# baek0203/multimodal_survival_prediction

Hardware: AMD Instinct MI355X
Metric: patients/sec per epoch (training epoch of the K-fold job: fwd + Cox + gate entropy + bwd + clip + Adam; HBM-resident cohort, batches gathered on the device inside the timed region -- the same epoch fed from pinned host memory over PCIe: config.h2d) (higher is better)
Workload: dtype f32

## Files before the change

### include/mmsurv.h

```cpp
#ifndef MMSURV_H
#define MMSURV_H
#include <stdint.h>
#include <stddef.h>

#ifndef HIP_INCLUDE_HIP_HIP_RUNTIME_API_H
typedef struct ihipStream_t* hipStream_t;
typedef struct ihipEvent_t* hipEvent_t;
#endif

#define MMS_OK 0
#define MMS_ERR_ARG (-1)
#define MMS_ERR_LAUNCH (-2)
#define MMS_MAX_GROUP 10

#ifdef __cplusplus
extern "C" {
#endif

typedef struct Dims3 { int D; int H; int W; } Dims3;

typedef struct MmsDnOpts {
    int out_features;
    int persist_b4;
    int persist_b3;
    int split_wgs;
    int conv1_ksplit;
    int conv1_small;
    int c1s_max_wgs;
    int conv1_small_bwd;
    int fuse_apply_rows;
    int conv3_small;
    int c3s_ring;
    int conv3_mt;
    int conv3_mt32_min;
    int conv3w_mt;
    int big_ng;
    int batch_w;
    int ms3_rows;
    int ms1_div;
    int c0_nwg;
    int c0f_nwg;
    int w2_packed;
    int trans_prepass;
    int fuse_layers;
    int wgrad_tab;
    int skip_dead_bwd;
    int c0_zero_skip;
    int dup_zero;
} MmsDnOpts;

typedef struct BnSrc {
    const double* sum;
    const double* sumsq;
    const float* rmean;
    const float* rvar;
    const float* gamma;
    const float* beta;
    float inv_count;
    float eps;
    int train;
    int nrep;
    int rep_stride;
} BnSrc;


typedef struct Conv1FwdP {
    const float* x; int ldx;
    int M;
    int K;
    const float* w;
    int N;
    float* y; int ldy;
    BnSrc bn;
    double* osum; double* osumsq;
    int pool;
    Dims3 in;
    int srep; int sstride;
    float* partial; int ksplit; unsigned* counters;
} Conv1FwdP;

typedef struct Conv3FwdP {
    const float* y1;
    const int* coords;
    Dims3 g; int M;
    const float* wp;
    float* out; int ldo;
    BnSrc bn;
    double* osum; double* osumsq;
    float* partial;
    int nsplit;
    int srep; int sstride;
    int wfrag;
    const unsigned* zwords; int zbps;
} Conv3FwdP;

typedef struct Conv0FwdP {
    const float* x;
    Dims3 in; Dims3 out;
    const int* coords;
    int M;
    const float* w;
    float* y;
    double* osum; double* osumsq;
    int srep; int sstride;
} Conv0FwdP;

typedef struct PoolFwdP {
    const float* y0; Dims3 in;
    Dims3 out; int B;
    float* slab; int ld;
    uint8_t* argmax;
    BnSrc bn;
    double* osum; double* osumsq;
    int srep; int sstride;
} PoolFwdP;

typedef struct PoolActP {
    const float* x; int ldx;
    int K;
    BnSrc bn;
    Dims3 in; int Mout;
    float* y; int ldy;
} PoolActP;

typedef struct HeadFwdP {
    const float* slab; int ld; int C; int B; int V;
    BnSrc bn;
    const float* w; const float* bias; int N;
    float* pooled;
    float* out; int ldo;
} HeadFwdP;

typedef struct BnBwd {
    const double* s1;
    const double* s2;
    int nrep; int rep_stride;
} BnBwd;

typedef struct Conv3BwdDataP {
    const float* dz; int lddz;
    const int* coords; Dims3 g; int M;
    const float* wpb;
    const float* y1;
    BnSrc bn;
    float* dbn;
    double* s1; double* s2;
    float* partial;
    int nsplit;
    int srep; int sstride;
    int wfrag;
    const unsigned* live;
} Conv3BwdDataP;

typedef struct Conv3BwdWP {
    const float* y1; const int* coords; Dims3 g; int M;
    BnSrc bn;
    const float* dz; int lddz;
    float* dw;
    int msplit;
    int dw_layout;
    const unsigned* live;
} Conv3BwdWP;

#define MMS_WGRAD_MAX_MODELS 5
#define MMS_WGRAD_MAX_MEMBERS 90
typedef struct MmsWgradModel {
    const void* tab;
    const float* slab;
    const float* dslab;
    const int* coords;
    const double* st_slab;
    int M; Dims3 g; int srep;
} MmsWgradModel;
typedef struct MmsWgradMember {
    float* dw2;
    float* dw1;
    float* dgamma2; float* dbeta2;
    int model; int layer;
} MmsWgradMember;
typedef struct MmsWgradShape {
    int ld; int C0;
    int ms3; int ms1;
    int dw_layout;
    int count;
} MmsWgradShape;

typedef struct Conv1BwdP {
    const float* dyraw; int lddy;
    const float* y; int ldy;
    BnSrc bn_out; BnBwd bb_out; int has_bn_out;
    int M; int N;
    const float* x; int ldx; int K; BnSrc bn_in;
    const float* w;
    int pool; Dims3 in;
    float* dw;
    float* dbn; int lddbn;
    double* s1; double* s2;
    int msplit;
    float* dgamma_out; float* dbeta_out;
    int srep; int sstride;
    float* fuse_dx; int fuse_lddx; int fuse_accumulate;
    float* fuse_dgamma; float* fuse_dbeta;
    const unsigned* live;
} Conv1BwdP;

typedef struct BnBwdApplyP {
    const float* dbn; int lddbn;
    const float* x; int ldx;
    float* dx; int lddx;
    int M; int C; BnSrc bn; BnBwd bb; int accumulate;
    float* dgamma; float* dbeta;
    const unsigned* live;
} BnBwdApplyP;

typedef struct HeadBwdP {
    const float* dout; int lddout;
    const float* pooled;
    const float* slab; int ld; int C; int B; int V; BnSrc bn;
    const float* w; int N;
    float* dw; float* dbias;
    float* dgamma; float* dbeta;
    float* dslab; int ldd;
    double* ext_sums;
} HeadBwdP;

typedef struct PoolBwdP {
    const float* dslab; int ld;
    const uint8_t* argmax; Dims3 out; Dims3 in; int B;
    const float* y0; BnSrc bn;
    float* dbn;
    double* s1; double* s2;
    const int* coords;
    int srep; int sstride;
} PoolBwdP;

typedef struct Conv0BwdWP {
    const float* dbn; const float* y0; BnSrc bn; BnBwd bb;
    const float* x; Dims3 in; Dims3 out; const int* coords; int M;
    float* dw; int msplit;
    float* dgamma; float* dbeta;
    float* dw_rep; int nrep;
    const unsigned* live;
} Conv0BwdWP;

typedef struct Conv0BwdDataP {
    const float* dbn;
    BnSrc bn;
    const float* w;
    Dims3 in; Dims3 out;
    int M;
    float* dx;
} Conv0BwdDataP;

typedef struct FbConvP {
    const float* x; int Cin; Dims3 in; Dims3 out; int B;
    int has_bn; BnSrc bn;
    const float* w; const float* bias; int Cout;
    float* y;
    double* osum; double* osumsq;
    const float* dy;
    float* dw; float* dbias;
    float* dbn_in; double* s1; double* s2;
    int msplit;
} FbConvP;

typedef struct FbPoolP {
    const float* y; int C; int V; int B; BnSrc bn;
    float* out; int ldo;
    const float* dout; int lddout;
    float* dbn; double* s1; double* s2;
} FbPoolP;

typedef struct InProlog {
    int bn;
    const float* gamma; const float* beta;
    float* rmean; float* rvar; long long* nbt;
    float eps; float momentum;
    int train;
    float drop_p;
    const float* drop_mask;
    const uint32_t* rng;
    uint32_t stream_id;
} InProlog;

typedef struct LinearFwdP {
    const float* x; int ldx; int M; int K;
    InProlog pro;
    const float* w; const float* bias; int N;
    float* y; int ldy; int out_relu;
} LinearFwdP;

typedef struct LinearBwdP {
    const float* dy; int lddy;
    const float* y; int ldy;
    int out_relu;
    const float* x; int ldx; int M; int K; InProlog pro;
    const float* w; int N;
    float* dw; float* dbias;
    float* dx; int lddx;
    float* dgamma; float* dbeta;
} LinearBwdP;

typedef struct GateP {
    const float* feats; const float* mask; int M;
    const float* w1; const float* b1; const float* w2; const float* b2;
    float* hidden;
    float* gate;
    float* fused;
    const float* dfused;
    float ent_weight;
    const float* dgate_ext;
    float* dfeats;
    float* dw1; float* db1; float* dw2; float* db2;
    float* entropy;
// ... 90 lines not shown
typedef struct AugRec {
    int flip;
    int dz; int dy; int dx;
    float scale; float offset;
    int drop;
    int reserved;
} AugRec;
#define MMS_AUG_PLAIN 0
#define MMS_AUG_VOLUME 1
#define MMS_AUG_MASK 2
typedef struct AugP {
    const AugRec* rec;
    int role[8];
    int drop_bit[8];
    int D; int H; int W;
    int max_shift[3];
} AugP;

typedef struct AffRec {
    float m[12];
    float sigma;
    unsigned seed;
    int reserved[2];
} AffRec;
typedef struct AffP {
    const AffRec* rec;
    int stage_floats;
} AffP;

int mms_abi_sizeof(const char* name);
int mms_abi_version(void);

int mms_init_coords(int* coords, int B, int D, int H, int W, hipStream_t s);
int mms_conv0_fwd(const Conv0FwdP* p, hipStream_t s);
int mms_pool_fwd(const PoolFwdP* p, hipStream_t s);
int mms_conv1_fwd(const Conv1FwdP* p, hipStream_t s);
int mms_conv3_fwd(const Conv3FwdP* p, hipStream_t s);
int mms_head_fwd(const HeadFwdP* p, hipStream_t s);
int mms_conv3_bwd_data(const Conv3BwdDataP* p, hipStream_t s);
int mms_conv3_bwd_weight(const Conv3BwdWP* p, hipStream_t s);
int mms_conv1_bwd_data(const Conv1BwdP* p, hipStream_t s);
int mms_conv1_bwd_weight(const Conv1BwdP* p, hipStream_t s);
int mms_bn_bwd_apply(const BnBwdApplyP* p, hipStream_t s);
int mms_head_bwd(const HeadBwdP* p, hipStream_t s);
int mms_pool_bwd(const PoolBwdP* p, hipStream_t s);
int mms_conv0_bwd_weight(const Conv0BwdWP* p, hipStream_t s);
int mms_unpack_conv3_grads(const void* table_host, int nlayers, hipStream_t s);
int mms_pack_conv3(const float* w, float* wpf, float* wpb, hipStream_t s);
int mms_pack_conv3_frag(const float* w, float* wff, float* wfb, hipStream_t s);
int mms_pack_conv3_table(const void* table_dev, int nlayers, hipStream_t s);
int mms_bn_running_update(const void* table_dev, int n, float momentum, hipStream_t s);


int mms_fb_conv_fwd(const FbConvP* p, hipStream_t s);
int mms_fb_conv_bwd_w(const FbConvP* p, hipStream_t s);
int mms_fb_conv_bwd_x(const FbConvP* p, hipStream_t s);
int mms_fb_pool_fwd(const FbPoolP* p, hipStream_t s);
int mms_fb_pool_bwd(const FbPoolP* p, hipStream_t s);
int mms_fb_workspace_bytes(int B, int D, int H, int W, size_t* bytes);
int mms_fb_init(void* ws, int B, int D, int H, int W, const void* const* buffers, hipStream_t s);
int mms_fb_forward(void* ws, int B, int D, int H, int W, const float* x, const void* const* params,
                   const void* const* buffers, float* out, int ldo, int train, hipStream_t s);
int mms_fb_backward(void* ws, int B, int D, int H, int W, const float* x, const void* const* params,
                    const float* dout, int lddout, void* const* grads, hipStream_t s);
int mms_fb3_workspace_bytes(const int* widths, int B, int D, int H, int W, size_t* bytes);
int mms_fb3_init(void* ws, size_t ws_bytes, const int* widths, int B, int D, int H, int W, const void* const* buffers, hipStream_t s);
int mms_fb3_forward(void* ws, size_t ws_bytes, const int* widths, int B, int D, int H, int W, const float* x, const void* const* params,
                    const void* const* buffers, float* out, int ldo, int train, hipStream_t s);
int mms_fb3_backward(void* ws, size_t ws_bytes, const int* widths, int B, int D, int H, int W, const float* x, const void* const* params,
                     const float* dout, int lddout, void* const* grads, hipStream_t s);

int mms_conv0_bwd_data(const Conv0BwdDataP* p, hipStream_t s);
int mms_conv0_bwd_data_group(const Conv0BwdDataP* p, int ng, hipStream_t s);
int mms_dn121_input_grad(void* ws, int B, int D, int H, int W, const float* x, const void* const* params, const void* const* buffers,
                         const float* dout, int lddout, float* dx, const MmsDnOpts* opts, hipStream_t s);
int mms_fb3_input_grad(void* ws, size_t ws_bytes, const int* widths, int B, int D, int H, int W, const float* x, const void* const* params,
                       const void* const* buffers, const float* dout, int lddout, float* dx, hipStream_t s);
int mms_dn121_input_grad_group(int ng, void* const* ws, int B, int D, int H, int W, const float* const* x, const void* const* const* params,
                               const void* const* const* buffers, const float* const* dout, int lddout, float* const* dx,
                               const MmsDnOpts* opts, hipStream_t s);
int mms_fb3_input_grad_group(int ng, void* const* ws, size_t ws_bytes, const int* widths, int B, int D, int H, int W, const float* const* x,
                             const void* const* const* params, const void* const* const* buffers, const float* const* dout, int lddout,
                             float* const* dx, hipStream_t s);

typedef struct EnsP {
    const float* x[10];
    int K; size_t n;
    float* mean; float* spread;
} EnsP;
int mms_ensemble_reduce(const EnsP* p, hipStream_t s);

int mms_linear_fwd(const LinearFwdP* p, hipStream_t s);
int mms_linear_bwd(const LinearBwdP* p, hipStream_t s);
int mms_gate_fwd(const GateP* p, hipStream_t s);
int mms_gate_bwd(const GateP* p, hipStream_t s);
int mms_gate_entropy(const float* gate, int M, float scale, float* loss, float* dgate, hipStream_t s);
int mms_linear_big_fwd(const LinBigP* p, hipStream_t s);
int mms_linear_big_bwd_w(const LinBigP* p, hipStream_t s);
int mms_linear_big_bwd_x(const LinBigP* p, hipStream_t s);
int mms_bn1d_bwd_apply(const LinBigP* p, hipStream_t s);
int mms_missing_mix_fwd(const MixP* p, hipStream_t s);
int mms_missing_mix_bwd(const MixP* p, hipStream_t s);
int mms_cox_fwd_bwd(const CoxP* p, hipStream_t s);
int mms_moe_fwd(const MoeP* p, hipStream_t s);
int mms_moe_bwd(const MoeP* p, hipStream_t s);
int mms_cindex_counts(const CindexP* p, hipStream_t s);
int mms_grad_sumsq(const AdamP* p, hipStream_t s);
int mms_clip_adam(const AdamP* p, hipStream_t s);
int mms_w2_pack(const AdamP* p, hipStream_t s);

int mms_ablation_build(void);
int mms_dn121_workspace_bytes(int B, int D, int H, int W, size_t* bytes);
int mms_dn121_region(int B, int D, int H, int W, const char* name, int index, size_t* off, size_t* bytes);
int mms_dn121_init(void* ws, int B, int D, int H, int W, const void* const* params, const void* const* buffers, const MmsDnOpts* opts, hipStream_t s);
int mms_dn121_w2_fragmask(int B, int D, int H, int W, const MmsDnOpts* opts, uint64_t* mask);
int mms_dn121_forward(void* ws, int B, int D, int H, int W, const float* x, const void* const* params,
                      const void* const* buffers, float* out, int ldo, int train, const MmsDnOpts* opts, hipStream_t s);
int mms_dn121_backward(void* ws, int B, int D, int H, int W, const float* x, const void* const* params,
                       const float* dout, int lddout, void* const* grads, const MmsDnOpts* opts, hipStream_t s);
typedef int (*mms_sync_fn)(void* user, double* base, int nrep, long rep_stride, int ncols, long pair_stride, hipStream_t s);
int mms_dn121_init_sync(void* ws, int B, int D, int H, int W, const void* const* params, const void* const* buffers, int bn_world,
                        const MmsDnOpts* opts, hipStream_t s);
int mms_dn121_forward_sync(void* ws, int B, int D, int H, int W, const float* x, const void* const* params,
                           const void* const* buffers, float* out, int ldo, int bn_world, mms_sync_fn hook, void* user,
                           const MmsDnOpts* opts, hipStream_t s);
int mms_dn121_backward_stage(void* ws, int B, int D, int H, int W, const float* x, const void* const* params,
                             const float* dout, int lddout, void* const* grads, int block_hi, int block_lo,
                             int bn_world, mms_sync_fn hook, void* user, const MmsDnOpts* opts, hipStream_t s);
int mms_head_bwd_sums(const HeadBwdP* p, hipStream_t s);
int mms_head_bwd_apply(const HeadBwdP* p, hipStream_t s);
int mms_dn121_backward_mt(void* ws, int B, int D, int H, int W, const float* x, const void* const* params,
                          const float* dout, int lddout, void* const* grads, const MmsDnOpts* opts, hipStream_t s, hipStream_t side,
                          hipEvent_t ev_fork, hipEvent_t ev_join);

int mms_ct_preprocess(const float* x, int inD, int inH, int inW, float* out, int oD, int oH, int oW, float* scratch, hipStream_t s);
int mms_rna_log_zscore(const float* counts, float* out, int n, int g, hipStream_t s);

int mms_conv0_fwd_group(const Conv0FwdP* p, int ng, const MmsDnOpts* opts, hipStream_t s);
int mms_conv0_fwd_group_zw(const Conv0FwdP* p, unsigned* const* zwords, int ng, const MmsDnOpts* opts, hipStream_t s);
int mms_pool_fwd_group(const PoolFwdP* p, int ng, hipStream_t s);
int mms_pool_act_group(const PoolActP* p, int ng, hipStream_t s);
int mms_conv1_fwd_group(const Conv1FwdP* p, int ng, const MmsDnOpts* opts, hipStream_t s);
int mms_conv3_fwd_group(const Conv3FwdP* p, int ng, const MmsDnOpts* opts, hipStream_t s);
int mms_head_fwd_group(const HeadFwdP* p, int ng, hipStream_t s);
int mms_conv3_bwd_data_group(const Conv3BwdDataP* p, int ng, const MmsDnOpts* opts, hipStream_t s);
int mms_conv3_bwd_weight_group(const Conv3BwdWP* p, int ng, const MmsDnOpts* opts, hipStream_t s);
int mms_conv3_bwd_weight_msplit(int M, int members, const MmsDnOpts* opts);
int mms_conv1_bwd_data_group(const Conv1BwdP* p, int ng, const MmsDnOpts* opts, hipStream_t s);
int mms_conv1_bwd_weight_group(const Conv1BwdP* p, int ng, hipStream_t s);
int mms_wgrad_tab_group(const MmsWgradModel* models, int nmodels, const MmsWgradMember* members, int nmembers,
                        const MmsWgradShape* shape, int which, hipStream_t s);
int mms_bn_bwd_apply_group(const BnBwdApplyP* p, int ng, hipStream_t s);
int mms_head_bwd_group(const HeadBwdP* p, int ng, hipStream_t s);
int mms_pool_bwd_group(const PoolBwdP* p, int ng, hipStream_t s);
int mms_conv0_bwd_weight_group(const Conv0BwdWP* p, int ng, const MmsDnOpts* opts, hipStream_t s);
int mms_pack_conv3_table_group(const void* const* tables_dev, int ng, int nlayers, hipStream_t s);
int mms_pack_conv3_table_group_ex(const void* const* tables_dev, int ng, int nlayers, uint64_t fragmask, hipStream_t s);
int mms_bn_running_update_group(const void* const* tables_dev, int ng, int n, float momentum, hipStream_t s);
int mms_missing_mix_fwd_group(const MixP* p, int ng, hipStream_t s);
int mms_missing_mix_bwd_group(const MixP* p, int ng, hipStream_t s);
int mms_gather_rows_group(const GatherP* p, int ng, hipStream_t s);
int mms_gather_aug_group(const GatherP* p, const AugP* a, int ng, hipStream_t s);
int mms_gather_affine_group(const GatherP* p, const AugP* a, const AffP* f, int ng, hipStream_t s);
int mms_unpack_conv3_grads_group(const float* const* scratch, float* const* const* dw, int ng, int nlayers, hipStream_t s);
int mms_zero_regions_group(void* const* regions_dev, int ng, size_t bytes, hipStream_t s);
int mms_linear_fwd_group(const LinearFwdP* p, int ng, hipStream_t s);
int mms_linear_bwd_group(const LinearBwdP* p, int ng, hipStream_t s);
int mms_gate_fwd_group(const GateP* p, int ng, hipStream_t s);
int mms_gate_bwd_group(const GateP* p, int ng, hipStream_t s);
int mms_cox_fwd_bwd_group(const CoxP* p, int ng, hipStream_t s);
int mms_moe_fwd_group(const MoeP* p, int ng, hipStream_t s);
int mms_moe_bwd_group(const MoeP* p, int ng, hipStream_t s);
int mms_grad_sumsq_group(const AdamP* p, int ng, hipStream_t s);
int mms_clip_adam_group(const AdamP* p, int ng, hipStream_t s);
int mms_w2_pack_group(const AdamP* p, int ng, hipStream_t s);
int mms_dn121_forward_group(int ng, void* const* ws, int B, int D, int H, int W, const float* const* x,
                            const void* const* const* params, const void* const* const* buffers, float* const* out,
                            int ldo, int train, const MmsDnOpts* opts, hipStream_t s);
int mms_dn121_backward_group(int ng, void* const* ws, int B, int D, int H, int W, const float* const* x,
                             const void* const* const* params, const float* const* dout, int lddout,
                             void* const* const* grads, const MmsDnOpts* opts, hipStream_t s);

int mms_fb_conv_fwd_group(const FbConvP* p, int ng, hipStream_t s);
int mms_fb_conv_bwd_w_group(const FbConvP* p, int ng, hipStream_t s);
int mms_fb_conv_bwd_x_group(const FbConvP* p, int ng, hipStream_t s);
int mms_fb_pool_fwd_group(const FbPoolP* p, int ng, hipStream_t s);
int mms_fb_pool_bwd_group(const FbPoolP* p, int ng, hipStream_t s);
int mms_fb_forward_group(int ng, void* const* ws, int B, int D, int H, int W, const float* const* x,
                         const void* const* const* params, const void* const* const* buffers, float* const* out,
                         int ldo, int train, hipStream_t s);
int mms_fb_backward_group(int ng, void* const* ws, int B, int D, int H, int W, const float* const* x,
                          const void* const* const* params, const float* const* dout, int lddout,
                          void* const* const* grads, hipStream_t s);
int mms_fb3_forward_group(int ng, void* const* ws, size_t ws_bytes, const int* widths, int B, int D, int H, int W, const float* const* x,
                          const void* const* const* params, const void* const* const* buffers, float* const* out,
                          int ldo, int train, hipStream_t s);
int mms_fb3_backward_group(int ng, void* const* ws, size_t ws_bytes, const int* widths, int B, int D, int H, int W, const float* const* x,
                           const void* const* const* params, const float* const* dout, int lddout,
                           void* const* const* grads, hipStream_t s);
int mms_img_tail_fwd_group(const FbPoolP* pool, const LinearFwdP* l1, const LinearFwdP* l2, int ng, hipStream_t s);
int mms_img_tail_bwd_group(const FbPoolP* pool, const LinearBwdP* l1, const LinearBwdP* l2, int ng, hipStream_t s);
int mms_img_forward_group(int ng, void* const* ws, size_t ws_bytes, const int* widths, int B, int D, int H, int W, const float* const* x,
                          const void* const* const* params, const void* const* const* buffers, float* const* out,
                          int ldo, int train, const LinearFwdP* l1, const LinearFwdP* l2, hipStream_t s);
int mms_img_backward_group(int ng, void* const* ws, size_t ws_bytes, const int* widths, int B, int D, int H, int W, const float* const* x,
                           const void* const* const* params, void* const* const* grads, const LinearBwdP* l1, const LinearBwdP* l2,
                           hipStream_t s);

#ifdef __cplusplus
}
#endif
#endif
```

### multimodal_survival_prediction_amd/csrc/common.h

```cpp
#pragma once
#include <utility>
#include <hip/hip_runtime.h>
#include <atomic>
#include <mutex>
#include <stdint.h>
#include <stdio.h>

#include "../../include/mmsurv.h"

typedef float f32x16 __attribute__((ext_vector_type(16)));
typedef float f32x4 __attribute__((ext_vector_type(4)));

template <class P> struct Grp { P p[MMS_MAX_GROUP]; int zdim; };
template <class P> static inline bool grp_fill(Grp<P>& a, const P* pp, int ng, int zdim) {
    if (!pp || ng < 1 || ng > MMS_MAX_GROUP) return false;
    for (int g = 0; g < ng; ++g) a.p[g] = pp[g];
    a.zdim = zdim;
    return true;
}
#define MMS_SINGLE(name, T) extern "C" int name(const T* p, hipStream_t s) { return name##_group(p, 1, s); }
#define MMS_SINGLE_O(name, T) extern "C" int name(const T* p, hipStream_t s) { return name##_group(p, 1, nullptr, s); }
static inline MmsDnOpts mms_opts(const MmsDnOpts* o) { return o ? *o : MmsDnOpts{}; }


__device__ __forceinline__ void xcd_place(int& gi, int& bx) {
    gi = blockIdx.z; bx = blockIdx.x;
    if ((gridDim.x & 7) != 0) return;
    const int k = blockIdx.x & 7, per = gridDim.x >> 3, ng = gridDim.z;
    if (ng > 1 && ng <= 8 && (8 % ng) == 0) {
        const int X = 8 / ng, slots = per * ng, slot = (blockIdx.x >> 3) + per * blockIdx.z;
        gi = k / X; bx = (k % X) * slots + slot;
    } else {
        bx = k * per + (blockIdx.x >> 3);
    }
}

__device__ __forceinline__ void xcd_place_parts(int& gi, int& bx, int& X, int& q, int& sl) {
    gi = blockIdx.z; bx = blockIdx.x; X = 1; q = 0; sl = blockIdx.x;
    if ((gridDim.x & 7) != 0) return;
    const int k = blockIdx.x & 7, per = gridDim.x >> 3, ng = gridDim.z;
    if (ng > 1 && ng <= 8 && (8 % ng) == 0) {
        X = 8 / ng; q = k % X; sl = (blockIdx.x >> 3) + per * blockIdx.z;
        gi = k / X; bx = q * (per * ng) + sl;
    } else {
        X = 8; q = k; sl = blockIdx.x >> 3;
        bx = k * per + sl;
    }
}

struct DupPlan { unsigned dups; int rep; };
__device__ __forceinline__ unsigned dup_issue(const unsigned* zw, int B) {
    const int lane = threadIdx.x & 63;
    return (zw && lane < B) ? __hip_atomic_load(zw + lane, __ATOMIC_RELAXED, __HIP_MEMORY_SCOPE_AGENT) : 0xffffffffu;
}
__device__ __forceinline__ bool dup_resolve(unsigned word, unsigned zbps, int B, int tps, int mode, int X, int q, int sl, int& tile, DupPlan& pl) {
    pl.dups = 0; pl.rep = 0;
    const unsigned zmask = (unsigned)__builtin_amdgcn_readfirstlane((int)(unsigned)__ballot(word == zbps));
    if (__popc(zmask) < 2) return true;
    const int rep = __ffs((int)zmask) - 1;
    const unsigned dmask = zmask & ~(1u << rep);
    int s;
    if (mode == 1) {
        s = tile / tps;
        if ((dmask >> s) & 1u) return false;
    } else {
        const int ct = (B - __popc(dmask)) * tps;
        if (sl * X + q >= ct) return false;
        const int t = q * (ct / X) + (q < ct % X ? q : ct % X) + sl;
        int cs = t / tps;
        for (s = 0; s < B; ++s) {
            if ((dmask >> s) & 1u) continue;
            if (cs == 0) break;
            --cs;
        }
        tile = s * tps + t % tps;
    }
    if (s == rep) { pl.dups = dmask; pl.rep = rep; }
    return true;
}

__device__ __forceinline__ unsigned live_issue(const unsigned* w) {
    return w ? __hip_atomic_load(w, __ATOMIC_RELAXED, __HIP_MEMORY_SCOPE_AGENT) : 1u;
}
__device__ __forceinline__ bool live_dead(unsigned v) { return __builtin_amdgcn_readfirstlane(v) == 0u; }
struct LiveTab { const unsigned* w[MMS_MAX_GROUP]; };
static inline LiveTab live_tab(const unsigned* const* live, int ng) {
    LiveTab t{};
    for (int g = 0; live && g < ng && g < MMS_MAX_GROUP; ++g) t.w[g] = live[g];
    return t;
}
template <class P, class = void> struct has_live_word { static constexpr bool value = false; };
template <class P> struct has_live_word<P, decltype((void)std::declval<const P&>().live)> { static constexpr bool value = true; };
template <class P> __device__ __forceinline__ const unsigned* live_word_of(const P& p) {
    if constexpr (has_live_word<P>::value) return p.live; else return nullptr;
}

__device__ __forceinline__ bool syncthreads_any(bool flag, int (*vote)[4], int& par) {
    const int w = __ballot(flag) != 0ull;
    if ((threadIdx.x & 63) == 0) vote[par][threadIdx.x >> 6] = w;
    __syncthreads();
    const int4 v = *(const int4*)vote[par];
    par ^= 1;
    return __builtin_amdgcn_readfirstlane(v.x | v.y | v.z | v.w) != 0;
}

template <class F, int... T>
__device__ __forceinline__ void static_for_impl(F&& f, std::integer_sequence<int, T...>) { (f(std::integral_constant<int, T>{}), ...); }
template <int N, class F>
__device__ __forceinline__ void static_for(F&& f) { static_for_impl(f, std::make_integer_sequence<int, N>{}); }

__device__ __forceinline__ double* stat_rep(double* base, int nrep, int stride) {
    return (base && nrep > 1) ? base + (size_t)(blockIdx.x % nrep) * stride : base;
}
template <int NA, class V>
__device__ __forceinline__ void rep_add(const V* const (&a)[NA], int nrep, size_t stride_doubles, V (&s)[NA]) {
    for (int r0 = 1; r0 < nrep; r0 += 3) {
        V t[NA][3];
#pragma unroll
        for (int j = 0; j < 3; ++j) {
            const size_t o = (size_t)(r0 + j < nrep ? r0 + j : 0) * stride_doubles;
#pragma unroll
            for (int i = 0; i < NA; ++i) t[i][j] = *(const V*)((const double*)a[i] + o);
        }
#pragma unroll
        for (int j = 0; j < 3; ++j)
            if (r0 + j < nrep) {
#pragma unroll
                for (int i = 0; i < NA; ++i) s[i] += t[i][j];
            }
    }
}
__device__ __forceinline__ double rep_sum(const double* a, int c, int nrep, int stride) {
    double s[1] = {a[c]};
    const double* const p[1] = {a + c};
    rep_add(p, nrep, (size_t)stride, s);
    return s[0];
}

__device__ __forceinline__ void pstore(float* p, float v) { __hip_atomic_store(p, v, __ATOMIC_RELAXED, __HIP_MEMORY_SCOPE_AGENT); }
__device__ __forceinline__ float pload(const float* p) { return __hip_atomic_load(p, __ATOMIC_RELAXED, __HIP_MEMORY_SCOPE_AGENT); }
__device__ __forceinline__ bool tile_last_arriver(unsigned* counter, unsigned nsplit, int tid) {
    __shared__ unsigned s_last;
    asm volatile("s_waitcnt vmcnt(0)" ::: "memory");
    __syncthreads();
    if (tid == 0) {
        const unsigned old = atomicAdd(counter, 1u);
        s_last = (old == nsplit - 1u) ? 1u : 0u;
        if (old == nsplit - 1u) atomicExch(counter, 0u);
    }
    __syncthreads();
    return s_last != 0u;
}

__device__ __forceinline__ void rep_sum2(const double* a, const double* b, int c, int nrep, int stride, double& sa, double& sb) {
    double s[2] = {a[c], b[c]};
    const double* const p[2] = {a + c, b + c};
    rep_add(p, nrep, (size_t)stride, s);
    sa = s[0]; sb = s[1];
}

__device__ __forceinline__ void bn_mean_rstd(const BnSrc& b, int c, float& mean, float& rstd) {
    if (!b.gamma) { mean = 0.f; rstd = 1.f; return; }
    if (b.train) {
        double s, q;
        rep_sum2(b.sum, b.sumsq, c, b.nrep, b.rep_stride, s, q);
        const double m = s * (double)b.inv_count;
        double v = q * (double)b.inv_count - m * m;
        v = v > 0.0 ? v : 0.0;
        mean = (float)m;
        rstd = 1.0f / sqrtf((float)v + b.eps);
    } else {
        mean = b.rmean[c];
        rstd = 1.0f / sqrtf(b.rvar[c] + b.eps);
    }
}

__device__ __forceinline__ void bn_consts1(const BnSrc& b, int c, float& mean, float& rstd, float& gamma, float& beta) {
    if (!b.gamma) { mean = 0.f; rstd = 1.f; gamma = 1.f; beta = 0.f; return; }
    gamma = b.gamma[c]; beta = b.beta[c];
    bn_mean_rstd(b, c, mean, rstd);
}

__device__ __forceinline__ void bn_bwd_consts(const BnSrc& b, const BnBwd& bb, int c, float& mean, float& rstd, float& gamma, double& t1, double& t2) {
    if (!b.train) {
        gamma = b.gamma[c]; mean = b.rmean[c]; rstd = 1.0f / sqrtf(b.rvar[c] + b.eps);
        t1 = 0.0; t2 = 0.0;
        return;
    }
    double sq[2] = {b.sum[c], b.sumsq[c]}, tt[2] = {bb.s1[c], bb.s2[c]};
    gamma = b.gamma[c];
    { const double* const p[2] = {b.sum + c, b.sumsq + c}; rep_add(p, b.nrep, (size_t)b.rep_stride, sq); }
    { const double* const p[2] = {bb.s1 + c, bb.s2 + c}; rep_add(p, bb.nrep, (size_t)bb.rep_stride, tt); }
    t1 = tt[0]; t2 = tt[1];
    const double s = sq[0], q = sq[1];
    const double m = s * (double)b.inv_count;
    double v = q * (double)b.inv_count - m * m;
    v = v > 0.0 ? v : 0.0;
    mean = (float)m;
    rstd = 1.0f / sqrtf((float)v + b.eps);
}

__device__ __forceinline__ void bn_consts4(const BnSrc& b, int c, float (&mean)[4], float (&sc)[4], float (&beta)[4]) {
    if (!b.gamma) {
#pragma unroll
        for (int i = 0; i < 4; ++i) { mean[i] = 0.f; sc[i] = 1.f; beta[i] = 0.f; }
        return;
    }
    const float4 g = *(const float4*)(b.gamma + c), be = *(const float4*)(b.beta + c);
    float4 mu4, rs4;
    if (b.train) {
        typedef double d2 __attribute__((ext_vector_type(2)));
        d2 sv[4] = {*(const d2*)(b.sum + c), *(const d2*)(b.sum + c + 2), *(const d2*)(b.sumsq + c), *(const d2*)(b.sumsq + c + 2)};
        { const d2* const p[4] = {(const d2*)(b.sum + c), (const d2*)(b.sum + c + 2), (const d2*)(b.sumsq + c), (const d2*)(b.sumsq + c + 2)};
          rep_add(p, b.nrep, (size_t)b.rep_stride, sv); }
        const d2 s01 = sv[0], s23 = sv[1], q01 = sv[2], q23 = sv[3];
        const double ic = (double)b.inv_count;
        const double m0 = s01.x * ic, m1 = s01.y * ic, m2 = s23.x * ic, m3 = s23.y * ic;
        const double v0 = q01.x * ic - m0 * m0, v1 = q01.y * ic - m1 * m1, v2 = q23.x * ic - m2 * m2, v3 = q23.y * ic - m3 * m3;
        mu4 = make_float4((float)m0, (float)m1, (float)m2, (float)m3);
        rs4 = make_float4(1.0f / sqrtf((float)(v0 > 0.0 ? v0 : 0.0) + b.eps), 1.0f / sqrtf((float)(v1 > 0.0 ? v1 : 0.0) + b.eps),
                          1.0f / sqrtf((float)(v2 > 0.0 ? v2 : 0.0) + b.eps), 1.0f / sqrtf((float)(v3 > 0.0 ? v3 : 0.0) + b.eps));
    } else {
        const float4 rv = *(const float4*)(b.rvar + c);
        mu4 = *(const float4*)(b.rmean + c);
        rs4 = make_float4(1.0f / sqrtf(rv.x + b.eps), 1.0f / sqrtf(rv.y + b.eps), 1.0f / sqrtf(rv.z + b.eps), 1.0f / sqrtf(rv.w + b.eps));
    }
    mean[0] = mu4.x; mean[1] = mu4.y; mean[2] = mu4.z; mean[3] = mu4.w;
    sc[0] = g.x * rs4.x; sc[1] = g.y * rs4.y; sc[2] = g.z * rs4.z; sc[3] = g.w * rs4.w;
    beta[0] = be.x; beta[1] = be.y; beta[2] = be.z; beta[3] = be.w;
}
static inline bool mms_bn_aligned16(const BnSrc& b) {
// ... 129 lines not shown
```

### multimodal_survival_prediction_amd/csrc/dn_bwd.hip

```cpp
#include "dn_ops.h"
#include "tile_gemm.h"
#include <string.h>
#include <stdlib.h>

#define Z4 make_float4(0, 0, 0, 0)

__device__ __forceinline__ unsigned tap_mask9(int c, Dims3 g, bool mirror) {
    int d, h, w;
    unpack_dhw(c, d, h, w);
    const unsigned lo_d = d > 0, hi_d = d + 1 < g.D, lo_h = h > 0, hi_h = h + 1 < g.H, lo_w = w > 0, hi_w = w + 1 < g.W;
    const unsigned dm = mirror ? (hi_d | 2u | (lo_d << 2)) : (lo_d | 2u | (hi_d << 2));
    const unsigned hm = mirror ? (hi_h | 2u | (lo_h << 2)) : (lo_h | 2u | (hi_h << 2));
    const unsigned wm = mirror ? (hi_w | 2u | (lo_w << 2)) : (lo_w | 2u | (hi_w << 2));
    return dm | (hm << 3) | (wm << 6);
}

__device__ __forceinline__ void store_tile_bwd(float* y, int M, int m0, const float* Cs, int tid) {
    for (int idx = tid; idx < 32 * 128; idx += 256) {
        const int r = idx >> 7, c = idx & 127, m = m0 + r;
        if (m < M) y[(size_t)m * 128 + c] = Cs[r * 129 + c];
    }
}

template <bool SPLIT>
// ... 10 lines not shown
    buf_rsrc_t rz, rw;
    __device__ void setup(const Params& p, int m0, int, int, float* extra, int tid) {
        ex = extra;
        p_nsplit = p.nsplit > 0 ? p.nsplit : 27;
        if (tid < 128) {
            float mu, rstd, ga_, be_;
            bn_consts1(p.bn, tid, mu, rstd, ga_, be_);
            extra[tid] = mu; extra[128 + tid] = rstd; extra[256 + tid] = ga_; extra[384 + tid] = be_;
        }
        rz = make_rsrc(p.dz, (unsigned)(p.M - 1) * (unsigned)p.lddz * 4u + 128u);
        rw = make_rsrc(p.wpb, 128u * 27u * 32u * 4u);
        const int row = tid >> 3, co = (tid & 7) * 4, m = m0 + row;
        const bool valid = m < p.M;
        m9 = valid ? tap_mask9(p.coords[valid ? m : m0], p.g, true) : 0u;
        voff = ((valid ? m : m0) * p.lddz + co) * 4;
#pragma unroll
        for (int i = 0; i < 4; ++i) woff[i] = (((tid >> 3) + 32 * i) * 864 + co) * 4;
    }
    __device__ void krange(const Params&, int z, int& kb, int& ke) {
        if (SPLIT) {
            const int tpw = (27 + p_nsplit - 1) / p_nsplit;
            kb = z * tpw * 32; ke = kb + tpw * 32; if (ke > 27 * 32) ke = 27 * 32;
        } else { kb = 0; ke = 27 * 32; }
    }
    __device__ void step(const Params& p, int k0) {
        const int tap = k0 >> 5, kd = tap / 9, kh = (tap / 3) % 3, kw = tap % 3;
        sel = (1u << kd) | (8u << kh) | (64u << kw);
        tapoff_b = -(((kd - 1) * p.g.H + (kh - 1)) * p.g.W + (kw - 1)) * p.lddz * 4;
        wsoff = k0 * 4;
    }
    __device__ float4 a_ld(const Params&, int, int, int, bool& ok) const {
        ok = (m9 & sel) == sel;
        return buf_load4(rz, voff + (ok ? tapoff_b : 0), 0);
    }
    __device__ float4 a_tx(const Params&, int, const float4& v, int, int, bool ok) const {
        const float z = ok ? 1.f : 0.f;
        return make_float4(z * v.x, z * v.y, z * v.z, z * v.w);
    }
    __device__ float4 b_ld(const Params&, int i, int, int, bool& ok) const { ok = true; return buf_load4(rw, woff[i], wsoff); }
    __device__ float4 b_tx(const Params&, int, const float4& v, int, int, bool) const { return v; }
    __device__ void epilogue(const Params& p, int m0_, int, int z, const float* Cs, int tid, bool active) {
        if (SPLIT) {
            if (active) store_tile_bwd(p.partial + (size_t)z * p.M * 128, p.M, m0_, Cs, tid);
            return;
        }
        const int c = tid & 127, rg = tid >> 7;
        const float mu = ex[c], rstd = ex[128 + c], ga = ex[256 + c], be = ex[384 + c];
        double s1 = 0, s2 = 0;
        const int rows = !active ? 0 : (p.M - m0_ < TM ? p.M - m0_ : TM);
        float yv[TM / 2];
#pragma unroll
        for (int i = 0; i < TM / 2; ++i) {
            const int r = rg + 2 * i;
            yv[i] = r < rows ? p.y1[(size_t)(m0_ + r) * 128 + c] : 0.f;
        }
#pragma unroll
        for (int i = 0; i < TM / 2; ++i) {
            const int r = rg + 2 * i;
            if (r < rows) {
                const float xh = (yv[i] - mu) * rstd;
                const float pre = fmaf(ga, xh, be);
                const float g = pre > 0.f ? Cs[r * (TN + 1) + c] : 0.f;
                p.dbn[(size_t)(m0_ + r) * 128 + c] = g;
                s1 += g; s2 += (double)g * xh;
            }
        }
        double* red = (double*)(ex + 544);
        if (active) { red[(rg * 2 + 0) * 128 + c] = s1; red[(rg * 2 + 1) * 128 + c] = s2; }
        __syncthreads();
        if (rg == 0 && active) {
            atomicAdd(&stat_rep(p.s1, p.srep, p.sstride)[c], red[c] + red[2 * 128 + c]);
            atomicAdd(&stat_rep(p.s2, p.srep, p.sstride)[c], red[128 + c] + red[3 * 128 + c]);
        }
    }
};

__global__ __launch_bounds__(256) void conv3_bwd_data_reduce_kernel(const Grp<Conv3BwdDataP> grp) {
    const Conv3BwdDataP& p = grp.p[blockIdx.z];
    const unsigned alive = live_issue(p.live);
    __shared__ double red[2][2][128];
    const int c = threadIdx.x & 127, rg = threadIdx.x >> 7;
    float mu, rstd;
    bn_mean_rstd(p.bn, c, mu, rstd);
    const float ga = p.bn.gamma[c], be = p.bn.beta[c];
    if (live_dead(alive)) return;
    double s1 = 0, s2 = 0;
    const int mend = blockIdx.x * 4 + 4 < p.M ? blockIdx.x * 4 + 4 : p.M;
    for (int m = blockIdx.x * 4 + rg; m < mend; m += 2) {
        float v[27];
#pragma unroll
        for (int t = 0; t < 27; ++t) v[t] = t < p.nsplit ? p.partial[((size_t)t * p.M + m) * 128 + c] : 0.f;
        float a = 0.f;
#pragma unroll
        for (int t = 0; t < 27; ++t) a += v[t];
        const size_t o = (size_t)m * 128 + c;
        const float xh = (p.y1[o] - mu) * rstd;
        const float g = fmaf(ga, xh, be) > 0.f ? a : 0.f;
        p.dbn[o] = g;
        s1 += g; s2 += (double)g * xh;
    }
    red[0][rg][c] = s1; red[1][rg][c] = s2;
    __syncthreads();
    if (rg == 0) {
        atomicAdd(&stat_rep(p.s1, p.srep, p.sstride)[c], red[0][0][c] + red[0][1][c]);
        atomicAdd(&stat_rep(p.s2, p.srep, p.sstride)[c], red[1][0][c] + red[1][1][c]);
    }
}

template <int RT>
__global__ __launch_bounds__(256) void conv3_bwd_data_reduce16_kernel(const Grp<Conv3BwdDataP> grp) {
    const Conv3BwdDataP& p = grp.p[blockIdx.z];
    const unsigned alive = live_issue(p.live);
    __shared__ double red[2][2][128];
    const int c = threadIdx.x & 127, rg = threadIdx.x >> 7;
    float mu, rstd;
    bn_mean_rstd(p.bn, c, mu, rstd);
    const float ga = p.bn.gamma[c], be = p.bn.beta[c];
    if (live_dead(alive)) return;
    const int m0 = blockIdx.x * (2 * RT) + rg;
    float v[RT][4], y[RT];
#pragma unroll
    for (int i = 0; i < RT; ++i) {
        const int m = m0 + 2 * i;
        const bool ok = m < p.M;
#pragma unroll
        for (int t = 0; t < 4; ++t) v[i][t] = (ok && t < p.nsplit) ? p.partial[((size_t)t * p.M + m) * 128 + c] : 0.f;
        y[i] = ok ? p.y1[(size_t)m * 128 + c] : 0.f;
    }
    double s1 = 0, s2 = 0;
#pragma unroll
    for (int i = 0; i < RT; ++i) {
        const int m = m0 + 2 * i;
        if (m < p.M) {
            float a = 0.f;
#pragma unroll
            for (int t = 0; t < 4; ++t) a += v[i][t];
            const float xh = (y[i] - mu) * rstd;
            const float g = fmaf(ga, xh, be) > 0.f ? a : 0.f;
            p.dbn[(size_t)m * 128 + c] = g;
            s1 += g; s2 += (double)g * xh;
        }
    }
    red[0][rg][c] = s1; red[1][rg][c] = s2;
    __syncthreads();
    if (rg == 0) {
        atomicAdd(&stat_rep(p.s1, p.srep, p.sstride)[c], red[0][0][c] + red[0][1][c]);
        atomicAdd(&stat_rep(p.s2, p.srep, p.sstride)[c], red[1][0][c] + red[1][1][c]);
    }
}

#define C3D_BP 36
#define C3D_MAXHALO 17
#define C3D_PIN() do { if constexpr (PIN) { asm volatile("" ::: "memory"); __builtin_amdgcn_sched_barrier(0); } } while (0)
template <bool PIN>
__global__ __launch_bounds__(256) __attribute__((amdgpu_waves_per_eu(3, 3))) void conv3_bwd_data_mt_kernel(const Grp<Conv3BwdDataP> grp) {
    int gi, bx;
    xcd_place(gi, bx);
    const Conv3BwdDataP& p = grp.p[gi];
    const unsigned alive = live_issue(p.live);
    const float* __restrict__ dz = p.dz;
    const float* __restrict__ wpb = p.wpb;
    const float* __restrict__ y1 = p.y1;
    float* __restrict__ dbn = p.dbn;
    const int M = p.M, lddz = p.lddz, W = p.g.W, HW = p.g.H * p.g.W;
    extern __shared__ __attribute__((aligned(16))) float smem[];
    const int tid = threadIdx.x, lane = tid & 63, wave = tid >> 6, li = lane & 31, kq = lane >> 5;
    const int m0 = bx * 32, halo = W + 1, nrows = 32 + 2 * halo;
    const int cin = 32 * wave + li;
    float mu, rstd, ga, be;
    bn_consts1(p.bn, cin, mu, rstd, ga, be);
    const int myrow = m0 + li;
    const int mycoord = p.coords[myrow < M ? myrow : 0];
    constexpr int NR = (32 + 2 * C3D_MAXHALO + 31) / 32;
    float4 wv[3][NR];
    const int wr = tid >> 3, wc = (tid & 7) * 4;
#pragma unroll
    for (int kd = 0; kd < 3; ++kd)
#pragma unroll
        for (int i = 0; i < NR; ++i) {
            const int r = wr + 32 * i, src = m0 - (kd - 1) * HW - halo + r;
            const bool ok = r < nrows && src >= 0 && src < M;
            const float4 v = *(const float4*)(dz + (size_t)(ok ? src : 0) * lddz + wc);
            wv[kd][i] = ok ? v : make_float4(0.f, 0.f, 0.f, 0.f);
        }
    const float* wl = wpb + (size_t)cin * 864 + 4 * kq;
    float4 b[3][4];
    auto bload = [&](float4 (&bb)[4], int tap) __attribute__((always_inline)) {
#pragma unroll
        for (int q = 0; q < 4; ++q) bb[q] = *(const float4*)(wl + tap * 32 + 8 * q);
    };
    bload(b[0], 0);
    bload(b[1], 1);
    if (live_dead(alive)) return;
#pragma unroll
    for (int kd = 0; kd < 3; ++kd)
#pragma unroll
        for (int i = 0; i < NR; ++i) {
            const int r = wr + 32 * i;
            if (r < nrows) *(float4*)&smem[(kd * nrows + r) * C3D_BP + wc] = wv[kd][i];
        }
    if (tid < C3D_BP) smem[3 * nrows * C3D_BP + tid] = 0.f;
    const unsigned m9 = myrow < M ? tap_mask9(mycoord, p.g, true) : 0u;
    __syncthreads();
    const float* arow = smem + (li + halo) * C3D_BP + 4 * kq;
    const float* azero = smem + 3 * nrows * C3D_BP + 4 * kq;
    f32x16 acc, acc2;
#pragma unroll
    for (int r = 0; r < 16; ++r) { acc[r] = 0.f; acc2[r] = 0.f; }
    float4 aL[2], aH[2];
    auto aread = [&](float4 (&a)[2], int tap, int half) __attribute__((always_inline)) {
        const int kd = tap / 9, t9 = tap - 9 * kd, kh = t9 / 3, kw = t9 - 3 * kh;
        const unsigned sel = (1u << kd) | (8u << kh) | (64u << kw);
        const float* ar = (m9 & sel) == sel ? arow + (kd * nrows - ((kh - 1) * W + (kw - 1))) * C3D_BP : azero;
#pragma unroll
        for (int q = 0; q < 2; ++q) a[q] = *(const float4*)(ar + 8 * (half * 2 + q));
    };
    auto mma = [&](const float4 (&a)[2], const float4 (&bb)[4], int half) __attribute__((always_inline)) {
#pragma unroll
        for (int q = 0; q < 2; ++q) {
            const float4& bq = bb[half * 2 + q];
            acc = __builtin_amdgcn_mfma_f32_32x32x2f32(a[q].x, bq.x, acc, 0, 0, 0);
            acc2 = __builtin_amdgcn_mfma_f32_32x32x2f32(a[q].y, bq.y, acc2, 0, 0, 0);
            acc = __builtin_amdgcn_mfma_f32_32x32x2f32(a[q].z, bq.z, acc, 0, 0, 0);
            acc2 = __builtin_amdgcn_mfma_f32_32x32x2f32(a[q].w, bq.w, acc2, 0, 0, 0);
        }
    };
    aread(aL, 0, 0);
    static_for<27>([&](auto T) __attribute__((always_inline)) {
        constexpr int tap = decltype(T)::value;
        if constexpr (tap + 2 < 27) bload(b[(tap + 2) % 3], tap + 2);
        aread(aH, tap, 1);
        C3D_PIN();
        mma(aL, b[tap % 3], 0);
        C3D_PIN();
        if constexpr (tap + 1 < 27) aread(aL, tap + 1, 0);
        C3D_PIN();
        mma(aH, b[tap % 3], 1);
        C3D_PIN();
    });
    float yv[16];
#pragma unroll
    for (int r = 0; r < 16; ++r) {
        const int m = m0 + 4 * kq + (r & 3) + 8 * (r >> 2);
        yv[r] = y1[(size_t)(m < M ? m : 0) * 128 + cin];
    }
    double s1 = 0, s2 = 0;
#pragma unroll
    for (int r = 0; r < 16; ++r) {
        const int m = m0 + 4 * kq + (r & 3) + 8 * (r >> 2);
        if (m < M) {
            const float xh = (yv[r] - mu) * rstd;
            const float pre = fmaf(ga, xh, be);
            const float g = pre > 0.f ? acc[r] + acc2[r] : 0.f;
            dbn[(size_t)m * 128 + cin] = g;
            s1 += g; s2 += (double)g * xh;
        }
    }
    s1 += __shfl_xor(s1, 32);
    s2 += __shfl_xor(s2, 32);
    if (kq == 0) {
        atomicAdd(&stat_rep(p.s1, p.srep, p.sstride)[cin], s1);
        atomicAdd(&stat_rep(p.s2, p.srep, p.sstride)[cin], s2);
    }
}
static inline bool conv3_bwd_data_mt_ok(int M, int ng, const Dims3& g, const MmsDnOpts& o) {
    if (g.W + 1 > C3D_MAXHALO || o.conv3_mt < 0) return false;
    if (o.conv3_mt == 2 || o.conv3_mt == 3) return M >= 64;
    const int min32 = o.conv3_mt32_min > 0 ? o.conv3_mt32_min : 256;
    return M >= 1024 && (long)((M + 31) / 32) * ng >= min32;
}
template <bool PIN>
static int launch_conv3_bwd_data_mt(const Conv3BwdDataP* pp, int ng, hipStream_t s) {
    const Conv3BwdDataP& p = *pp;
    const int smem = (3 * (32 + 2 * (p.g.W + 1)) + 1) * C3D_BP * (int)sizeof(float);
    Grp<Conv3BwdDataP> a;
    grp_fill(a, pp, ng, 1);
    MMS_LAUNCH((conv3_bwd_data_mt_kernel<PIN>), dim3((p.M + 31) / 32, 1, ng), dim3(256), smem, s, a);
    return mms_check_launch();
}

extern "C" int mms_conv3_bwd_data_group(const Conv3BwdDataP* pp, int ng, const MmsDnOpts* opts, hipStream_t s) {
    if (!pp || ng < 1 || ng > MMS_MAX_GROUP) return MMS_ERR_ARG;
    const MmsDnOpts o = mms_opts(opts);
    const Conv3BwdDataP& p = *pp;
    if (p.M <= 0 || p.lddz % 4 != 0) return MMS_ERR_ARG;
    for (int g = 1; g < ng; ++g) {
        const Conv3BwdDataP& q = pp[g];
        if (q.M != p.M || q.lddz % 4 != 0 || q.g.D != p.g.D || q.g.H != p.g.H || q.g.W != p.g.W ||
            (q.partial == nullptr) != (p.partial == nullptr) || q.nsplit != p.nsplit) return MMS_ERR_ARG;
    }
    for (int g = 1; g < ng; ++g) if (pp[g].wfrag != p.wfrag) return MMS_ERR_ARG;
    if (p.wfrag) return (!p.partial && mms_conv3_small_jn(p.M, ng, p.g, o)) ? mms_c3s_bwd_data(pp, ng, o, s) : MMS_ERR_ARG;
    if (p.partial) {
        if (p.nsplit < 1 || p.nsplit > 27 || (p.nsplit - 1) * ((27 + p.nsplit - 1) / p.nsplit) >= 27) return MMS_ERR_ARG;
        int rc = launch_tile_gemm<Conv3BwdDataOp<true>>(pp, ng, dim3((p.M + 31) / 32, 1, p.nsplit), s);
        if (rc != MMS_OK) return rc;
        Grp<Conv3BwdDataP> a;
        grp_fill(a, pp, ng, 1);
        if (p.nsplit <= 4 && p.M >= 512) MMS_LAUNCH(conv3_bwd_data_reduce16_kernel<8>, dim3((p.M + 15) / 16, 1, ng), dim3(256), 0, s, a);
        else MMS_LAUNCH(conv3_bwd_data_reduce_kernel, dim3((p.M + 3) / 4, 1, ng), dim3(256), 0, s, a);
        return mms_check_launch();
    }
    if (conv3_bwd_data_mt_ok(p.M, ng, p.g, o)) {
        for (int g = 0; g < ng; ++g) if (pp[g].lddz % 4 != 0 || ((uintptr_t)pp[g].dz & 15) != 0) return MMS_ERR_ARG;
        return (long)((p.M + 31) / 32) * ng <= 768 ? launch_conv3_bwd_data_mt<true>(pp, ng, s) : launch_conv3_bwd_data_mt<false>(pp, ng, s);
    }
    if (mms_conv3_small_jn(p.M, ng, p.g, o)) return mms_c3s_bwd_data(pp, ng, o, s);
    return launch_tile_gemm<Conv3BwdDataOp<false>>(pp, ng, dim3((p.M + 31) / 32, 1, 1), s);
}
MMS_SINGLE_O(mms_conv3_bwd_data, Conv3BwdDataP)

struct Conv3BwdWOp {
    typedef Conv3BwdWP Params;
    static constexpr int WM = 4, WN = 1, WK = 1, AMODE = LD_R4, BMODE = LD_R4;
    static constexpr int TM = 128, TN = 32;
    static constexpr int EXTRA = 1024;
    typedef float4 ARaw;
    typedef float4 BRaw;
    float mean[4], sc[4], beta[4];
    const unsigned* vm;
    int tap, mb, me, avoff[4], bvoff, tapoff_b, asoff, bsoff, k0s;
    unsigned sel;
    buf_rsrc_t ry, rz;
    static __device__ void zremap(int flat, int zdim, int nflat, int& gi, int& z) {
        const int pairs = nflat / 27, ms = zdim / 27;
        if ((pairs & 7) == 0) {
            const int x = flat & 7, slot = flat >> 3, pair = (slot / 27) * 8 + x;
            gi = pair / ms;
            z = (pair - gi * ms) * 27 + slot % 27;
        } else { gi = flat / zdim; z = flat - gi * zdim; }
    }
    __device__ void setup(const Params& p, int, int, int z, float* extra, int tid) {
        const int c0 = (tid & 31) * 4;
        bn_consts4(p.bn, c0, mean, sc, beta);
        tap = z % 27;
        const int kd = tap / 9, kh = (tap / 3) % 3, kw = tap % 3;
        sel = (1u << kd) | (8u << kh) | (64u << kw);
        tapoff_b = (((kd - 1) * p.g.H + (kh - 1)) * p.g.W + (kw - 1)) * 512;
        const int chunk = z / 27;
        int mc = (p.M + p.msplit - 1) / p.msplit;
        mc = (mc + 31) & ~31;
        mb = chunk * mc;
        me = mb + mc < p.M ? mb + mc : p.M;
        vm = (const unsigned*)extra;
        for (int j = tid; j < mc; j += 256) ((unsigned*)extra)[j] = (mb + j < me) ? tap_mask9(p.coords[mb + j], p.g, false) : 0u;
        ry = make_rsrc(p.y1, (unsigned)p.M * 512u);
        rz = make_rsrc(p.dz, (unsigned)(p.M - 1) * (unsigned)p.lddz * 4u + 128u);
#pragma unroll
        for (int i = 0; i < 4; ++i) avoff[i] = (((tid >> 5) + 8 * i) * 128 + c0) * 4;
        bvoff = ((tid >> 3) * p.lddz + (tid & 7) * 4) * 4;
    }
    __device__ void krange(const Params&, int, int& kb, int& ke) { kb = mb; ke = me; }
    __device__ void step(const Params& p, int k0) { k0s = k0; asoff = k0 * 512; bsoff = k0 * p.lddz * 4; }
    __device__ float4 a_ld(const Params&, int i, int, int, bool& ok) const {
        const unsigned mk = vm[k0s - mb + (threadIdx.x >> 5 & 7) + 8 * i];
        ok = (mk & sel) == sel;
        return buf_load4(ry, avoff[i] + asoff + (ok ? tapoff_b : 0), 0);
    }
    __device__ float4 a_tx(const Params&, int, const float4& v, int, int, bool ok) const {
        const float z = ok ? 1.f : 0.f;
        return make_float4(z * fmaxf(bn_apply(v.x, mean[0], sc[0], beta[0]), 0.f), z * fmaxf(bn_apply(v.y, mean[1], sc[1], beta[1]), 0.f),
                           z * fmaxf(bn_apply(v.z, mean[2], sc[2], beta[2]), 0.f), z * fmaxf(bn_apply(v.w, mean[3], sc[3], beta[3]), 0.f));
    }
    __device__ float4 b_ld(const Params&, int, int, int m, bool& ok) const {
        ok = m < me;
        return buf_load4(rz, bvoff, bsoff);
    }
    __device__ float4 b_tx(const Params&, int, const float4& v, int, int, bool ok) const {
        const float z = ok ? 1.f : 0.f;
        return make_float4(z * v.x, z * v.y, z * v.z, z * v.w);
    }
    __device__ void epilogue(const Params& p, int, int, int, const float* Cs, int tid, bool active) {
        if (mb >= me || !active) return;
#ifdef MMS_ABLATE_FLUSH
        if (p.M > 0) return;
#endif
        for (int idx = tid; idx < TM * TN; idx += 256) {
            const int cin = idx & 127, co = idx >> 7;
            const size_t dst = p.dw_layout == 2 ? ((size_t)co * 27 + tap) * 128 + cin : (p.dw_layout == 1 ? ((size_t)tap * 32 + co) * 128 + cin : ((size_t)co * 128 + cin) * 27 + tap);
            atomicAdd(&p.dw[dst], Cs[cin * (TN + 1) + co]);
        }
    }
};

struct UnpackTable { UnpackEntry e[64]; };
__global__ __launch_bounds__(256) void unpack_conv3_grads_kernel(const UnpackTable tab) {
    __shared__ float t[27 * 129];
    const UnpackEntry e = tab.e[blockIdx.y];
    const int co = blockIdx.x;
    for (int idx = threadIdx.x; idx < 27 * 128; idx += 256) {
        const int tap = idx >> 7, cin = idx & 127;
        t[tap * 129 + cin] = e.scratch[((size_t)tap * 32 + co) * 128 + cin];
    }
    __syncthreads();
    float* dst = e.dw + (size_t)co * 128 * 27;
    for (int idx = threadIdx.x; idx < 27 * 128; idx += 256) {
        const int cin = idx / 27, tap = idx % 27;
        dst[idx] += t[tap * 129 + cin];
    }
}
#define UNPACK_MAXG 7
struct UnpackGroup { const float* scratch[UNPACK_MAXG]; float* dw[UNPACK_MAXG][58]; const unsigned* live[UNPACK_MAXG]; };
__global__ __launch_bounds__(256) void unpack_conv3_grads_group_kernel(const UnpackGroup tab) {
    __shared__ float t[27 * 129];
    const int co = blockIdx.x, layer = blockIdx.y, g = blockIdx.z;
    if (live_dead(live_issue(tab.live[g]))) return;
    const float* scratch = tab.scratch[g] + (size_t)layer * 27 * 32 * 128;
    for (int idx = threadIdx.x; idx < 27 * 128; idx += 256) {
        const int tap = idx >> 7, cin = idx & 127;
        t[tap * 129 + cin] = scratch[((size_t)tap * 32 + co) * 128 + cin];
    }
    __syncthreads();
    float* dst = tab.dw[g][layer] + (size_t)co * 128 * 27;
    for (int idx = threadIdx.x; idx < 27 * 128; idx += 256) {
        const int cin = idx / 27, tap = idx % 27;
        dst[idx] += t[tap * 129 + cin];
    }
}
extern "C" int mms_unpack_conv3_grads_group_live(const float* const* scratch, float* const* const* dw, const unsigned* const* live, int ng, int nlayers, hipStream_t s) {
    if (nlayers <= 0) return MMS_OK;
    if (!scratch || !dw || ng < 1 || ng > MMS_MAX_GROUP || nlayers > 58) return MMS_ERR_ARG;
    for (int g0 = 0; g0 < ng; g0 += UNPACK_MAXG) {
        const int n = ng - g0 < UNPACK_MAXG ? ng - g0 : UNPACK_MAXG;
        UnpackGroup t;
        for (int g = 0; g < n; ++g) {
            t.scratch[g] = scratch[g0 + g];
            t.live[g] = live ? live[g0 + g] : nullptr;
            for (int i = 0; i < nlayers; ++i) t.dw[g][i] = dw[g0 + g][i];
        }
        MMS_LAUNCH(unpack_conv3_grads_group_kernel, dim3(32, nlayers, n), dim3(256), 0, s, t);
        const int rc = mms_check_launch();
        if (rc != MMS_OK) return rc;
    }
    return MMS_OK;
}
extern "C" int mms_unpack_conv3_grads_group(const float* const* scratch, float* const* const* dw, int ng, int nlayers, hipStream_t s) {
    return mms_unpack_conv3_grads_group_live(scratch, dw, nullptr, ng, nlayers, s);
}
extern "C" int mms_unpack_conv3_grads(const void* table_host, int nlayers, hipStream_t s) {
    if (nlayers <= 0) return MMS_OK;
    if (nlayers > 64) return MMS_ERR_ARG;
    UnpackTable t;
    memcpy(t.e, table_host, sizeof(UnpackEntry) * nlayers);
    MMS_LAUNCH(unpack_conv3_grads_kernel, dim3(32, nlayers), dim3(256), 0, s, t);
    return mms_check_launch();
}

#define C3W_AP 132
#define C3W_BP 36
#define C3W_STAGE (34 * C3W_AP + 32 * C3W_BP)
__global__ __launch_bounds__(256) __attribute__((amdgpu_waves_per_eu(2, 3))) void conv3_bwdw_mt_kernel(const Grp<Conv3BwdWP> grp) {
    int gi, z;
    {
        const int flat = blockIdx.z, nflat = gridDim.z, zdim = grp.zdim, pairs = nflat / 9, ms = zdim / 9;
        if ((pairs & 7) == 0) {
            const int x = flat & 7, slot = flat >> 3, pair = (slot / 9) * 8 + x;
            gi = pair / ms;
            z = (pair - gi * ms) * 9 + slot % 9;
        } else { gi = flat / zdim; z = flat - gi * zdim; }
    }
    const Conv3BwdWP& p = grp.p[gi];
    const unsigned alive = live_issue(p.live);
    extern __shared__ __attribute__((aligned(16))) float smem[];
    float2* vf = (float2*)(smem + 2 * C3W_STAGE);
    const int tid = threadIdx.x, lane = tid & 63, wave = tid >> 6, li = lane & 31, h = lane >> 5;
    const int kdh = z % 9, chunk = z / 9, kd = kdh / 3, kh = kdh - 3 * kd;
    const int offdh = ((kd - 1) * p.g.H + (kh - 1)) * p.g.W;
    int mc = (p.M + p.msplit - 1) / p.msplit;
    mc = (mc + 31) & ~31;
    const int mb = chunk * mc, me = mb + mc < p.M ? mb + mc : p.M;
    if (mb >= me) return;
    const int c0 = (tid & 31) * 4;
    float mean[4], sc[4], beta[4];
    bn_consts4(p.bn, c0, mean, sc, beta);
    if (live_dead(alive)) return;
    for (int j = tid; j < mc; j += 256) {
        const unsigned mk = (mb + j < me) ? tap_mask9(p.coords[mb + j], p.g, false) : 0u;
        vf[j] = make_float2(mk & 64u ? 1.f : 0.f, mk & 256u ? 1.f : 0.f);
    }
    const unsigned selb = (1u << kd) | (8u << kh);

    float4 ra[5], rb;
    unsigned oka = 0;
    bool okb = false;
    auto gload = [&](int r0) __attribute__((always_inline)) {
        oka = 0;
#pragma unroll
        for (int i = 0; i < 5; ++i) {
            const int j = (tid >> 5) + 8 * i, src = r0 + j - 1 + offdh;
            const bool ok = j < 34 && src >= 0 && src < p.M;
            oka |= (ok ? 1u : 0u) << i;
            ra[i] = ok ? *(const float4*)(p.y1 + (size_t)src * 128 + c0) : make_float4(0.f, 0.f, 0.f, 0.f);
        }
        const int m = r0 + (tid >> 3);
        rb = m < me ? *(const float4*)(p.dz + (size_t)m * p.lddz + (tid & 7) * 4) : make_float4(0.f, 0.f, 0.f, 0.f);
        okb = m < me && (tap_mask9(p.coords[m], p.g, false) & selb) == selb;
    };
    auto sstore = [&](float* st) __attribute__((always_inline)) {
#pragma unroll
        for (int i = 0; i < 5; ++i) {
            const int j = (tid >> 5) + 8 * i;
            if (j < 34) {
                const float zf = (oka >> i) & 1u ? 1.f : 0.f;
                *(float4*)&st[j * C3W_AP + c0] =
                    make_float4(zf * fmaxf(bn_apply(ra[i].x, mean[0], sc[0], beta[0]), 0.f), zf * fmaxf(bn_apply(ra[i].y, mean[1], sc[1], beta[1]), 0.f),
                                zf * fmaxf(bn_apply(ra[i].z, mean[2], sc[2], beta[2]), 0.f), zf * fmaxf(bn_apply(ra[i].w, mean[3], sc[3], beta[3]), 0.f));
            }
        }
        const float zb = okb ? 1.f : 0.f;
        *(float4*)&st[34 * C3W_AP + (tid >> 3) * C3W_BP + (tid & 7) * 4] = make_float4(zb * rb.x, zb * rb.y, zb * rb.z, zb * rb.w);
    };
    f32x16 acc0, acc1, acc2;
#pragma unroll
    for (int r = 0; r < 16; ++r) { acc0[r] = 0.f; acc1[r] = 0.f; acc2[r] = 0.f; }
    auto mma = [&](const float* st, int t) __attribute__((always_inline)) {
        const float* at = st + h * C3W_AP + 32 * wave + li;
        const float* bt = st + 34 * C3W_AP + h * C3W_BP + li;
        const float2* vt = vf + 32 * t + h;
        float a[33];
#ifdef C3W_NO_READ
#pragma unroll
        for (int j = 0; j < 33; ++j) a[j] = (float)(j + t);
#else
#pragma unroll
        for (int j = 0; j < 33; ++j) a[j] = at[j * C3W_AP];
#endif
#pragma unroll
        for (int q = 0; q < 16; ++q) {
            const int kk = 2 * q;
#ifdef C3W_NO_READ
            const float b = (float)(q + t);
            const float2 f = make_float2((float)(t & 1), 1.f);
#else
            const float b = bt[kk * C3W_BP];
            const float2 f = vt[kk];
#endif
#ifdef C3W_NO_MFMA
            acc0[q] += a[kk] * (b * f.x);
            acc1[q] += a[kk + 1] * b;
            acc2[q] += a[kk + 2] * (b * f.y);
#else
            acc0 = __builtin_amdgcn_mfma_f32_32x32x2f32(a[kk], b * f.x, acc0, 0, 0, 0);
            acc1 = __builtin_amdgcn_mfma_f32_32x32x2f32(a[kk + 1], b, acc1, 0, 0, 0);
            acc2 = __builtin_amdgcn_mfma_f32_32x32x2f32(a[kk + 2], b * f.y, acc2, 0, 0, 0);
#endif
        }
    };
    const int T = (me - mb + 31) / 32;
    gload(mb);
    sstore(smem);
    __syncthreads();
#pragma unroll 1
    for (int t = 0; t < T; ++t) {
        float* cur = smem + (t & 1) * C3W_STAGE;
        float* nxt = smem + ((t + 1) & 1) * C3W_STAGE;
#ifndef C3W_NO_LOAD
        if (t + 1 < T) gload(mb + 32 * (t + 1));
#endif
        mma(cur, t);
#ifndef C3W_NO_LOAD
        if (t + 1 < T) sstore(nxt);
#endif
#ifndef C3W_NO_BARRIER
        __syncthreads();
#endif
    }
    float* Cs = smem;
#pragma unroll
    for (int kw = 0; kw < 3; ++kw) {
        const f32x16& acc = kw == 0 ? acc0 : (kw == 1 ? acc1 : acc2);
#pragma unroll
        for (int r = 0; r < 16; ++r) Cs[(32 * wave + 4 * h + (r & 3) + 8 * (r >> 2)) * 33 + li] = acc[r];
        __syncthreads();
        const int tap = kdh * 3 + kw;
        for (int idx = tid; idx < 128 * 32; idx += 256) {
            const int cin = idx & 127, co = idx >> 7;
            const size_t dst = p.dw_layout == 2 ? ((size_t)co * 27 + tap) * 128 + cin : (p.dw_layout == 1 ? ((size_t)tap * 32 + co) * 128 + cin : ((size_t)co * 128 + cin) * 27 + tap);
            atomicAdd(&p.dw[dst], Cs[cin * 33 + co]);
        }
        __syncthreads();
    }
}
static inline bool conv3w_mt_ok(int rows_per_chunk, int msplit, int ng, const MmsDnOpts& o) {
    if (o.conv3w_mt < 0) return false;
    if (o.conv3w_mt == 2) return true;
    return rows_per_chunk >= 512 && mms_conv3w_mt_fills((long)msplit * ng * 9);
}

extern "C" int mms_conv3_bwd_weight_group(const Conv3BwdWP* pp, int ng, const MmsDnOpts* opts, hipStream_t s) {
    if (!pp || ng < 1 || ng > MMS_MAX_GROUP) return MMS_ERR_ARG;
    const MmsDnOpts o = mms_opts(opts);
    const Conv3BwdWP& p = *pp;
    if (p.M <= 0 || p.msplit <= 0 || p.lddz % 4 != 0 || p.dw_layout < 0 || p.dw_layout > 2) return MMS_ERR_ARG;
    if ((((p.M + p.msplit - 1) / p.msplit + 31) & ~31) > 1024) return MMS_ERR_ARG;
    for (int g = 0; g < ng; ++g) if (!mms_bn_aligned16(pp[g].bn)) return MMS_ERR_ARG;
    for (int g = 1; g < ng; ++g) {
        const Conv3BwdWP& q = pp[g];
        if (q.M != p.M || q.msplit != p.msplit || q.lddz % 4 != 0 || q.g.D != p.g.D || q.g.H != p.g.H || q.g.W != p.g.W ||
            q.dw_layout != p.dw_layout) return MMS_ERR_ARG;
    }
    if (conv3w_mt_ok(((p.M + p.msplit - 1) / p.msplit + 31) & ~31, p.msplit, ng, o)) {
        constexpr int smem = (2 * C3W_STAGE + 2 * 1024) * (int)sizeof(float);
        Grp<Conv3BwdWP> a;
        if (!grp_fill(a, pp, ng, 9 * p.msplit)) return MMS_ERR_ARG;
        MMS_LAUNCH(conv3_bwdw_mt_kernel, dim3(1, 1, 9 * p.msplit * ng), dim3(256), smem, s, a);
        return mms_check_launch();
    }
    return launch_tile_gemm<Conv3BwdWOp>(pp, ng, dim3(1, 1, 27 * p.msplit), s);
}
MMS_SINGLE_O(mms_conv3_bwd_weight, Conv3BwdWP)
extern "C" int mms_conv3_bwd_weight_msplit(int M, int members, const MmsDnOpts* opts) {
    if (M <= 0 || members < 1 || members > MMS_MAX_GROUP) return 0;
    return mms_conv3w_msplit(M, members, mms_opts(opts));
}

struct DyConsts {
    float *A, *Bc, *Cc, *mean, *rstd;
    __device__ void init(const Conv1BwdP& p, float* e, int n0, int cnt, int tid) {
        A = e; Bc = e + cnt; Cc = e + 2 * cnt; mean = e + 3 * cnt; rstd = e + 4 * cnt;
        if (!p.has_bn_out) return;
        for (int i = tid; i < cnt; i += 256) {
            const int n = n0 + i;
            if (n < p.N) {
                float mu, rs, ga;
                double t1, t2;
                bn_bwd_consts(p.bn_out, p.bb_out, n, mu, rs, ga, t1, t2);
                A[i] = ga * rs;
                Bc[i] = (float)(t1 * (double)p.bn_out.inv_count);
                Cc[i] = (float)(t2 * (double)p.bn_out.inv_count);
                mean[i] = mu; rstd[i] = rs;
            } else {
                A[i] = Bc[i] = Cc[i] = mean[i] = rstd[i] = 0.f;
            }
        }
    }
    __device__ __forceinline__ float dy(const Conv1BwdP& p, float g, float y, int i) const {
        if (!p.has_bn_out) return g;
        return A[i] * (g - Bc[i] - (y - mean[i]) * rstd[i] * Cc[i]);
    }
};

template <int WM_, int WN_, int WK_, bool POOL, bool ONE_ = false>
struct Conv1BwdDataOp {
    typedef Conv1BwdP Params;
    static constexpr bool ONE_TILE = ONE_;
    static constexpr bool SINGLE_BUF = WK_ == 4;
    static constexpr int WM = WM_, WN = WN_, WK = WK_, AMODE = LD_K4, BMODE = LD_R4;
    __device__ void step(const Params&, int) {}
    static constexpr int TM = 32 * WM, TN = 32 * WN;
    static constexpr int EXTRA = 5 * 128 + 4 * TN + TM + 1024;
    DyConsts dc;
    float* ein;
    const int* srcbase;
    int m0;
    __device__ void setup(const Params& p, int m0_, int n0, int, float* extra, int tid) {
        m0 = m0_;
        dc.init(p, extra, 0, 128, tid);
        ein = extra + 640;
        srcbase = (const int*)(extra + 640 + 4 * TN);
        if (tid < TN) {
            const int k = n0 + tid;
            float mu = 0, rs = 0, ga = 0, be = 0;
            if (k < p.K) bn_consts1(p.bn_in, k, mu, rs, ga, be);
            ein[tid] = mu; ein[TN + tid] = rs; ein[2 * TN + tid] = ga; ein[3 * TN + tid] = be;
        }
        if (POOL && tid < TM) {
            int m = m0 + tid, base = -1;
            if (m < p.M) {
                int D2 = p.in.D >> 1, H2 = p.in.H >> 1, W2 = p.in.W >> 1, vox2 = D2 * H2 * W2;
                int b = m / vox2, r = m % vox2, d = r / (H2 * W2), h = (r / W2) % H2, w = r % W2;
                base = ((b * p.in.D + 2 * d) * p.in.H + 2 * h) * p.in.W + 2 * w;
            }
            ((int*)extra)[640 + 4 * TN + tid] = base;
        }
    }
    __device__ void krange(const Params& p, int, int& kb, int& ke) { kb = 0; ke = p.N; }
    struct ARaw { float4 g, y; };
    typedef float4 BRaw;
    __device__ ARaw a_ld(const Params& p, int, int m, int n, bool& ok) const {
        ARaw r; r.y = Z4;
        ok = m < p.M && n < p.N;
        const size_t mm = m < p.M ? m : p.M - 1;
        const int nn = n < p.N ? n : p.N - 4;
        r.g = *(const float4*)(p.dyraw + mm * p.lddy + nn);
        if (p.has_bn_out) r.y = *(const float4*)(p.y + mm * p.ldy + nn);
        return r;
    }
    __device__ float4 a_tx(const Params& p, int, const ARaw& r, int, int n, bool ok) const {
        if (!ok) return Z4;
        if (!p.has_bn_out) return r.g;
        return make_float4(dc.dy(p, r.g.x, r.y.x, n), dc.dy(p, r.g.y, r.y.y, n + 1), dc.dy(p, r.g.z, r.y.z, n + 2), dc.dy(p, r.g.w, r.y.w, n + 3));
    }
    __device__ float4 b_ld(const Params& p, int, int k, int n, bool& ok) const {
        ok = n < p.N && k < p.K;
        return *(const float4*)(p.w + (size_t)(n < p.N ? n : p.N - 1) * p.K + (k < p.K ? k : p.K - 4));
    }
    __device__ float4 b_tx(const Params&, int, const float4& v, int, int, bool ok) const { return ok ? v : Z4; }
    __device__ void epilogue(const Params& p, int m0_, int n0, int, const float* Cs, int tid, bool active) {
        constexpr int RG = 256 / TN;
        const int c = tid % TN, rg = tid / TN, k = n0 + c;
        const float mu = ein[c], rs = ein[TN + c], ga = ein[2 * TN + c], be = ein[3 * TN + c];
        double s1 = 0, s2 = 0;
        const int rows = !active ? 0 : (p.M - m0_ < TM ? p.M - m0_ : TM);
        constexpr int NI = TM / RG;
        float xv[NI], gv[NI];
        if (!POOL) {
#pragma unroll
            for (int i = 0; i < NI; ++i) {
                const int r = rg + i * RG;
                xv[i] = (r < rows && k < p.K) ? p.x[(size_t)(m0_ + r) * p.ldx + k] : 0.f;
            }
#pragma unroll
            for (int i = 0; i < NI; ++i) {
                const int r = rg + i * RG;
                const bool ok = r < rows && k < p.K;
                const float xh = (xv[i] - mu) * rs;
                const float g = ok && fmaf(ga, xh, be) > 0.f ? Cs[r * (TN + 1) + c] : 0.f;
                gv[i] = g;
                if (ok && !p.fuse_dx) p.dbn[(size_t)(m0_ + r) * p.lddbn + k] = g;
                if (ok) { s1 += g; s2 += (double)g * xh; }
            }
        } else if (k < p.K) {
            for (int r = rg; r < rows; r += RG) {
                const float da = Cs[r * (TN + 1) + c];
                {
                    const int base = srcbase[r], HW = p.in.H * p.in.W, W = p.in.W;
                    const float d8 = da * 0.125f;
#pragma unroll
                    for (int o = 0; o < 8; ++o) {
                        const size_t src = base + (o >> 2) * HW + ((o >> 1) & 1) * W + (o & 1);
                        const float xh = (p.x[src * p.ldx + k] - mu) * rs;
                        const float g = fmaf(ga, xh, be) > 0.f ? d8 : 0.f;
                        p.dbn[src * p.lddbn + k] = g;
                        s1 += g; s2 += (double)g * xh;
                    }
                }
            }
        }
        double* red = (double*)(ein + 4 * TN + TM);
        if (active) { red[(rg * 2 + 0) * TN + c] = s1; red[(rg * 2 + 1) * TN + c] = s2; }
        __syncthreads();
        if (!POOL && p.fuse_dx) {
            if (k < p.K && active) {
                double a = 0, b = 0;
                for (int g = 0; g < RG; ++g) { a += red[(g * 2) * TN + c]; b += red[(g * 2 + 1) * TN + c]; }
                const float gr = ga * rs, m1 = (float)(a * (double)p.bn_in.inv_count), m2 = rs * (float)(b * (double)p.bn_in.inv_count);
                float ov[NI];
#pragma unroll
                for (int i = 0; i < NI; ++i) {
                    const int r = rg + i * RG;
                    ov[i] = (r < rows && p.fuse_accumulate) ? p.fuse_dx[(size_t)(m0_ + r) * p.fuse_lddx + k] : 0.f;
                }
#pragma unroll
                for (int i = 0; i < NI; ++i) {
                    const int r = rg + i * RG;
                    if (r < rows) p.fuse_dx[(size_t)(m0_ + r) * p.fuse_lddx + k] = ov[i] + gr * (gv[i] - m1 - (xv[i] - mu) * m2);
                }
                if (rg == 0 && p.fuse_dgamma) { p.fuse_dgamma[k] += (float)b; p.fuse_dbeta[k] += (float)a; }
// ... 203 lines not shown
    if (!models || !members || !shape || nmodels < 1 || nmodels > MMS_WGRAD_MAX_MODELS || nmembers < 1 || nmembers > MMS_WGRAD_MAX_MEMBERS ||
        which < 1 || which > 3) return MMS_ERR_ARG;
    const MmsWgradShape& sh = *shape;
    const MmsWgradModel& m0 = models[0];
    if (m0.M <= 0 || sh.ms3 <= 0 || sh.ms1 <= 0 || sh.count <= 0 || sh.ld % 4 != 0 || sh.C0 % 32 != 0 || sh.C0 < 32 || sh.ld < sh.C0 + 32 ||
        sh.dw_layout < 0 || sh.dw_layout > 2 || m0.srep < 1) return MMS_ERR_ARG;
    if ((((m0.M + sh.ms3 - 1) / sh.ms3 + 31) & ~31) > 1024) return MMS_ERR_ARG;
    if ((long)sh.ms3 * 27 * nmembers > 65535 || (long)sh.ms1 * nmembers > 65535) return MMS_ERR_ARG;
    for (int g = 0; g < nmodels; ++g) {
        const MmsWgradModel& q = models[g];
        if (!q.tab || !q.slab || !q.dslab || !q.coords || !q.st_slab) return MMS_ERR_ARG;
        if (q.M != m0.M || q.srep != m0.srep || q.g.D != m0.g.D || q.g.H != m0.g.H || q.g.W != m0.g.W) return MMS_ERR_ARG;
        if ((((uintptr_t)q.slab | (uintptr_t)q.dslab | (uintptr_t)q.st_slab) & 15) != 0) return MMS_ERR_ARG;
    }
    int kmax = 0;
    for (int i = 0; i < nmembers; ++i) {
        const MmsWgradMember& q = members[i];
        if (q.model < 0 || q.model >= nmodels || q.layer < 0 || sh.C0 + 32 * q.layer + 32 > sh.ld) return MMS_ERR_ARG;
        if (((which & 1) && !q.dw2) || ((which & 2) && (!q.dw1 || !q.dgamma2 || !q.dbeta2))) return MMS_ERR_ARG;
        if (sh.C0 + 32 * q.layer > kmax) kmax = sh.C0 + 32 * q.layer;
    }
    WgradTab t;
    memset(&t, 0, sizeof(t));
    for (int g = 0; g < nmodels; ++g) { t.mod[g] = models[g]; t.live[g] = live ? live[g] : nullptr; }
    for (int i = 0; i < nmembers; ++i) t.mem[i] = members[i];
    t.sh = sh; t.inv_count = 1.0f / (float)sh.count;
    if (which & 1) {
        constexpr size_t smem = TileGemmCfg<Conv3BwdWOp>::smem_bytes();
        static_assert(smem <= 64 * 1024, "no dynamic-LDS attribute needed");
        MMS_LAUNCH(wgrad_tab_conv3_kernel, dim3(1, 1, 27 * sh.ms3 * nmembers), dim3(256), smem, s, t);
        const int rc = mms_check_launch();
        if (rc != MMS_OK) return rc;
    }
    if (which & 2) {
        constexpr size_t smem = TileGemmCfg<Conv1BwdWOp<false>>::smem_bytes();
        static_assert(smem <= 64 * 1024, "no dynamic-LDS attribute needed");
        MMS_LAUNCH(wgrad_tab_conv1_kernel, dim3(2, (kmax + 63) / 64, sh.ms1 * nmembers), dim3(256), smem, s, t);
        const int rc = mms_check_launch();
        if (rc != MMS_OK) return rc;
    }
    return MMS_OK;
}

__global__ __launch_bounds__(256) void bn_bwd_apply_kernel(const Grp<BnBwdApplyP> grp, const int rows) {
    const BnBwdApplyP& p = grp.p[blockIdx.z];
    const unsigned alive = live_issue(p.live);
    __shared__ float cm[4][256];
    const int tid = threadIdx.x, c0 = blockIdx.y * 256;
    const int nc = p.C - c0 < 256 ? p.C - c0 : 256;
    if (tid < nc) {
        const int c = c0 + tid;
        float mu, rs, ga;
        double t1, t2;
        bn_bwd_consts(p.bn, p.bb, c, mu, rs, ga, t1, t2);
        cm[0][tid] = mu; cm[1][tid] = ga * rs;
        cm[2][tid] = (float)(t1 * (double)p.bn.inv_count);
        cm[3][tid] = rs * (float)(t2 * (double)p.bn.inv_count);
        if (blockIdx.x == 0 && p.dgamma) {
            p.dgamma[c] += (float)t2;
            p.dbeta[c] += (float)t1;
        }
    }
    if (live_dead(alive)) return;
    __syncthreads();
    const int nq = nc >> 2, rpar = 256 / nq;
    const int q = tid % nq, rl = tid / nq;
    if (rl >= rpar) return;
    const int c = 4 * q;
    const float4 mu = *(const float4*)&cm[0][c], gr = *(const float4*)&cm[1][c], m1 = *(const float4*)&cm[2][c], m2 = *(const float4*)&cm[3][c];
    const int r0 = blockIdx.x * rows, rend = r0 + rows < p.M ? r0 + rows : p.M;
    for (int rb = r0 + rl; rb < rend; rb += 4 * rpar) {
        float4 g[4], x[4], o[4];
#pragma unroll
        for (int j = 0; j < 4; ++j) {
            const int r = rb + j * rpar;
            const size_t m = r < rend ? r : rb;
            g[j] = *(const float4*)(p.dbn + m * p.lddbn + c0 + c);
            x[j] = *(const float4*)(p.x + m * p.ldx + c0 + c);
            o[j] = p.accumulate ? *(const float4*)(p.dx + m * p.lddx + c0 + c) : make_float4(0, 0, 0, 0);
        }
#pragma unroll
        for (int j = 0; j < 4; ++j) {
            const int r = rb + j * rpar;
            if (r < rend) {
                float4 v = o[j];
                v.x += gr.x * (g[j].x - m1.x - (x[j].x - mu.x) * m2.x);
                v.y += gr.y * (g[j].y - m1.y - (x[j].y - mu.y) * m2.y);
                v.z += gr.z * (g[j].z - m1.z - (x[j].z - mu.z) * m2.z);
                v.w += gr.w * (g[j].w - m1.w - (x[j].w - mu.w) * m2.w);
                *(float4*)(p.dx + (size_t)r * p.lddx + c0 + c) = v;
            }
        }
    }
}

extern "C" int mms_bn_bwd_apply_group(const BnBwdApplyP* pp, int ng, hipStream_t s) {
    Grp<BnBwdApplyP> a;
    if (!grp_fill(a, pp, ng, 1)) return MMS_ERR_ARG;
    const BnBwdApplyP& p = *pp;
    if (p.M <= 0 || p.C <= 0 || p.C % 4 != 0 || p.lddbn % 4 || p.ldx % 4 || p.lddx % 4) return MMS_ERR_ARG;
    for (int g = 1; g < ng; ++g) {
        const BnBwdApplyP& q = pp[g];
        if (q.M != p.M || q.C != p.C || q.lddbn % 4 || q.ldx % 4 || q.lddx % 4 || q.accumulate != p.accumulate) return MMS_ERR_ARG;
    }
    const int rows = (long)p.M * ng >= 16384 ? 128 : 32;
    MMS_LAUNCH(bn_bwd_apply_kernel, dim3((p.M + rows - 1) / rows, (p.C + 255) / 256, ng), dim3(256), 0, s, a, rows);
    return mms_check_launch();
}
MMS_SINGLE(mms_bn_bwd_apply, BnBwdApplyP)

__global__ __launch_bounds__(256) void head_bwd_feat_kernel(const Grp<HeadBwdP> grp) {
    const HeadBwdP& p = grp.p[blockIdx.z];
    __shared__ double red[2][4][64];
    const int cl = threadIdx.x & 63, bl = threadIdx.x >> 6, c = blockIdx.x * 64 + cl;
    const bool ok = c < p.C;
    float mu = 0.f, rs = 0.f, ga = 0.f, be = 0.f;
    if (ok) bn_consts1(p.bn, c, mu, rs, ga, be);
    const int M = p.B * p.V;
    const float invV = 1.f / (float)p.V;
    double s1 = 0, s2 = 0;
    if (ok)
        for (int b = bl; b < p.B; b += 4) {
            float dp = 0;
#pragma unroll 16
            for (int n = 0; n < p.N; ++n) dp = fmaf(p.dout[b * p.lddout + n], p.w[(size_t)n * p.C + c], dp);
            dp *= invV;
            for (int v = 0; v < p.V; ++v) {
                const size_t m = (size_t)b * p.V + v;
                const float xh = (p.slab[m * p.ld + c] - mu) * rs;
                const float g = fmaf(ga, xh, be) > 0.f ? dp : 0.f;
                p.dslab[m * p.ldd + c] = g;
                s1 += g; s2 += (double)g * xh;
            }
        }
    red[0][bl][cl] = s1; red[1][bl][cl] = s2;
    __syncthreads();
    if (!ok) return;
    const double t1 = red[0][0][cl] + red[0][1][cl] + red[0][2][cl] + red[0][3][cl];
    const double t2 = red[1][0][cl] + red[1][1][cl] + red[1][2][cl] + red[1][3][cl];
    const float m1 = (float)(t1 / M), m2 = (float)(t2 / M);
    for (int b = bl; b < p.B; b += 4)
        for (int v = 0; v < p.V; ++v) {
            const size_t m = (size_t)b * p.V + v;
            const float xh = (p.slab[m * p.ld + c] - mu) * rs;
            const float g = p.dslab[m * p.ldd + c];
            p.dslab[m * p.ldd + c] = ga * rs * (g - m1 - xh * m2);
        }
    if (bl == 0) {
        p.dgamma[c] += (float)t2;
        p.dbeta[c] += (float)t1;
    }
}
#define HEAD_LIVE_SCAN 16384
__global__ __launch_bounds__(256) void head_bwd_w_kernel(const Grp<HeadBwdP> grp, const LiveTab lt) {
    const HeadBwdP& p = grp.p[blockIdx.z];
    unsigned* const live_out = (unsigned*)lt.w[blockIdx.z];
    if (blockIdx.x == 0 && live_out) {
        const int n_el = p.B * p.N;
        int any = n_el > HEAD_LIVE_SCAN;
        if (!any) for (int i = threadIdx.x; i < n_el; i += 256) any |= p.dout[(i / p.N) * p.lddout + i % p.N] != 0.0f;
        any = __syncthreads_or(any);
        if (threadIdx.x == 0) __hip_atomic_store(live_out, any ? 1u : 0u, __ATOMIC_RELAXED, __HIP_MEMORY_SCOPE_AGENT);
    }
    const int idx = blockIdx.x * 256 + threadIdx.x;
    if (idx >= p.N * p.C) return;
    const int n = idx / p.C, c = idx % p.C;
    float a = 0;
    for (int b = 0; b < p.B; ++b) a = fmaf(p.dout[b * p.lddout + n], p.pooled[b * p.C + c], a);
    p.dw[idx] += a;
    if (c == 0) {
        float d = 0;
        for (int b = 0; b < p.B; ++b) d += p.dout[b * p.lddout + n];
        p.dbias[n] += d;
    }
}
extern "C" int mms_head_bwd_group(const HeadBwdP* pp, int ng, hipStream_t s) { return mms_head_bwd_group_live(pp, nullptr, ng, s); }
extern "C" int mms_head_bwd_group_live(const HeadBwdP* pp, unsigned* const* live_out, int ng, hipStream_t s) {
    Grp<HeadBwdP> a;
    if (!grp_fill(a, pp, ng, 1)) return MMS_ERR_ARG;
    const HeadBwdP& p = *pp;
    if (p.B <= 0) return MMS_ERR_ARG;
    for (int g = 1; g < ng; ++g) {
        const HeadBwdP& q = pp[g];
        if (q.B != p.B || q.C != p.C || q.N != p.N || q.V != p.V) return MMS_ERR_ARG;
    }
    MMS_LAUNCH(head_bwd_feat_kernel, dim3((p.C + 63) / 64, 1, ng), dim3(256), 0, s, a);
    MMS_LAUNCH(head_bwd_w_kernel, dim3((p.N * p.C + 255) / 256, 1, ng), dim3(256), 0, s, a, live_tab((const unsigned* const*)live_out, ng));
    return mms_check_launch();
}
MMS_SINGLE(mms_head_bwd, HeadBwdP)

__global__ __launch_bounds__(256) void head_bwd_sums_kernel(const HeadBwdP p) {
    const int c = blockIdx.x * 256 + threadIdx.x;
    if (c >= p.C) return;
    float mu, rs, ga, be;
    bn_consts1(p.bn, c, mu, rs, ga, be);
    const float invV = 1.f / (float)p.V;
    double s1 = 0, s2 = 0;
    for (int b = 0; b < p.B; ++b) {
        float dp = 0;
        for (int n = 0; n < p.N; ++n) dp = fmaf(p.dout[b * p.lddout + n], p.w[(size_t)n * p.C + c], dp);
        dp *= invV;
        for (int v = 0; v < p.V; ++v) {
            const size_t m = (size_t)b * p.V + v;
            const float xh = (p.slab[m * p.ld + c] - mu) * rs;
            const float g = fmaf(ga, xh, be) > 0.f ? dp : 0.f;
            p.dslab[m * p.ldd + c] = g;
            s1 += g; s2 += (double)g * xh;
        }
    }
    p.ext_sums[c] = s1; p.ext_sums[p.C + c] = s2;
}
__global__ __launch_bounds__(256) void head_bwd_apply_kernel(const HeadBwdP p) {
    const int c = blockIdx.x * 256 + threadIdx.x;
    if (c >= p.C) return;
    float mu, rs;
    bn_mean_rstd(p.bn, c, mu, rs);
    const float ga = p.bn.gamma[c];
    const double t1 = p.ext_sums[c], t2 = p.ext_sums[p.C + c];
    const float m1 = (float)(t1 * (double)p.bn.inv_count), m2 = (float)(t2 * (double)p.bn.inv_count);
    for (int m = 0; m < p.B * p.V; ++m) {
        const float xh = (p.slab[(size_t)m * p.ld + c] - mu) * rs;
        const float g = p.dslab[(size_t)m * p.ldd + c];
        p.dslab[(size_t)m * p.ldd + c] = ga * rs * (g - m1 - xh * m2);
    }
    p.dgamma[c] += (float)t2;
    p.dbeta[c] += (float)t1;
}
extern "C" int mms_head_bwd_sums(const HeadBwdP* pp, hipStream_t s) {
    if (!pp || pp->B <= 0 || !pp->ext_sums) return MMS_ERR_ARG;
    MMS_LAUNCH(head_bwd_sums_kernel, dim3((pp->C + 255) / 256), dim3(256), 0, s, *pp);
    return mms_check_launch();
}
extern "C" int mms_head_bwd_apply(const HeadBwdP* pp, hipStream_t s) {
    if (!pp || pp->B <= 0 || !pp->ext_sums) return MMS_ERR_ARG;
    Grp<HeadBwdP> a;
    if (!grp_fill(a, pp, 1, 1)) return MMS_ERR_ARG;
    MMS_LAUNCH(head_bwd_apply_kernel, dim3((pp->C + 255) / 256), dim3(256), 0, s, *pp);
    MMS_LAUNCH(head_bwd_w_kernel, dim3((pp->N * pp->C + 255) / 256, 1, 1), dim3(256), 0, s, a, LiveTab{});
    return mms_check_launch();
}

__global__ __launch_bounds__(256) void pool_bwd_kernel(const Grp<PoolBwdP> grp, const LiveTab lt) {
    const PoolBwdP& p = grp.p[blockIdx.z];
    const unsigned alive = live_issue(lt.w[blockIdx.z]);
    __shared__ double red[2][4][64];
    const int c = threadIdx.x & 63, vr = threadIdx.x >> 6;
    float mu, rs, ga, be;
    bn_consts1(p.bn, c, mu, rs, ga, be);
    if (live_dead(alive)) return;
    const int vox_in = p.in.D * p.in.H * p.in.W, Min = p.B * vox_in, vox_out = p.out.D * p.out.H * p.out.W;
    double s1 = 0, s2 = 0;
    for (int it = 0; it < 16; ++it) {
        const int m = blockIdx.x * 64 + it * 4 + vr;
        if (m >= Min) break;
        int b, id, ih, iw;
        if (p.coords) {
            unpack_dhw(p.coords[m], id, ih, iw);
            b = (m - ((id * p.in.H + ih) * p.in.W + iw)) / vox_in;
        } else {
            const int r = m % vox_in;
            b = m / vox_in; id = r / (p.in.H * p.in.W); ih = (r / p.in.W) % p.in.H; iw = r % p.in.W;
        }
        const float y = p.y0[(size_t)m * 64 + c];
        uint8_t am[8];
        float gv[8];
#pragma unroll
        for (int k = 0; k < 8; ++k) {
            const int od = min((id + (k >> 2)) >> 1, p.out.D - 1), oh = min((ih + ((k >> 1) & 1)) >> 1, p.out.H - 1),
                      ow = min((iw + (k & 1)) >> 1, p.out.W - 1);
            const size_t mo = (size_t)b * vox_out + ((size_t)od * p.out.H + oh) * p.out.W + ow;
            am[k] = p.argmax[mo * 64 + c];
            gv[k] = p.dslab[mo * p.ld + c];
        }
        float g = 0.f;
#pragma unroll
        for (int k = 0; k < 8; ++k) {
            const int kd = k >> 2, kh = (k >> 1) & 1, kw = k & 1;
            const int od = (id + kd) >> 1, oh = (ih + kh) >> 1, ow = (iw + kw) >> 1;
            const bool ok = (kd == 0 || (id & 1)) && (kh == 0 || (ih & 1)) && (kw == 0 || (iw & 1)) &&
                            od < p.out.D && oh < p.out.H && ow < p.out.W;
            const int tap = ((id - 2 * od + 1) * 3 + (ih - 2 * oh + 1)) * 3 + (iw - 2 * ow + 1);
            g += (ok && am[k] == tap) ? gv[k] : 0.f;
        }
        const float xh = (y - mu) * rs;
        g = fmaf(ga, xh, be) > 0.f ? g : 0.f;
        p.dbn[(size_t)m * 64 + c] = g;
        s1 += g; s2 += (double)g * xh;
    }
    red[0][vr][c] = s1; red[1][vr][c] = s2;
    __syncthreads();
    if (vr == 0) {
        atomicAdd(&stat_rep(p.s1, p.srep, p.sstride)[c], red[0][0][c] + red[0][1][c] + red[0][2][c] + red[0][3][c]);
        atomicAdd(&stat_rep(p.s2, p.srep, p.sstride)[c], red[1][0][c] + red[1][1][c] + red[1][2][c] + red[1][3][c]);
    }
}
template <int WT>
__global__ __launch_bounds__(256) void pool_bwd_brick_kernel(const Grp<PoolBwdP> grp, const LiveTab lt) {
    const PoolBwdP& p = grp.p[blockIdx.z];
    const unsigned alive = live_issue(lt.w[blockIdx.z]);
    constexpr int WO = WT / 2 + 1, NC = 2 * 3 * WO;
    __shared__ float cg[NC][64];
    __shared__ uint8_t ca[NC][64];
    __shared__ double red[2][4][64];
    const int c = threadIdx.x & 63, vr = threadIdx.x >> 6;
    const int Di = p.in.D, Hi = p.in.H, Wi = p.in.W, Do = p.out.D, Ho = p.out.H, Wo = p.out.W;
    const int nwt = Wi / WT, nhb = Hi / 4, ndb = Di / 2;
    int r = blockIdx.x;
    const int wt = r % nwt; r /= nwt;
    const int hb = r % nhb; r /= nhb;
    const int db = r % ndb, b = r / ndb;
    const int w0 = wt * WT, ow0 = w0 >> 1;
    for (int cand = vr; cand < NC; cand += 4) {
        const int dd = cand / (3 * WO), hh = (cand / WO) % 3, ww = cand % WO;
        const int od = db + dd, oh = 2 * hb + hh, ow = ow0 + ww;
        const bool ok = od < Do && oh < Ho && ow < Wo;
        const size_t mo = ok ? ((size_t)(b * Do + od) * Ho + oh) * Wo + ow : 0;
        cg[cand][c] = ok ? p.dslab[mo * p.ld + c] : 0.f;
        ca[cand][c] = ok ? p.argmax[mo * 64 + c] : (uint8_t)255;
    }
    float mu, rs, ga, be;
    bn_consts1(p.bn, c, mu, rs, ga, be);
    if (live_dead(alive)) return;
    __syncthreads();
    double s1 = 0, s2 = 0;
    for (int v = vr; v < 8 * WT; v += 4) {
        const int di = v / (4 * WT), hi = (v / WT) & 3, wi = v % WT;
        const int id = 2 * db + di, ih = 4 * hb + hi, iw = w0 + wi;
        const size_t m = ((size_t)(b * Di + id) * Hi + ih) * Wi + iw;
        const float y = p.y0[m * 64 + c];
        float g = 0.f;
#pragma unroll
        for (int k = 0; k < 8; ++k) {
            const int kd = k >> 2, kh = (k >> 1) & 1, kw = k & 1;
            const int dd = (di + kd) >> 1, hh = (hi + kh) >> 1, ww = (wi + kw) >> 1;
            const int od = db + dd, oh = 2 * hb + hh, ow = ow0 + ww;
            const bool ok = (kd == 0 || (id & 1)) && (kh == 0 || (ih & 1)) && (kw == 0 || (iw & 1));
            const int tap = ((id - 2 * od + 1) * 3 + (ih - 2 * oh + 1)) * 3 + (iw - 2 * ow + 1);
            const int cand = (dd * 3 + hh) * WO + ww;
            g += (ok && ca[cand][c] == tap) ? cg[cand][c] : 0.f;
        }
        const float xh = (y - mu) * rs;
        g = fmaf(ga, xh, be) > 0.f ? g : 0.f;
        p.dbn[m * 64 + c] = g;
        s1 += g; s2 += (double)g * xh;
    }
    red[0][vr][c] = s1; red[1][vr][c] = s2;
    __syncthreads();
    if (vr == 0) {
        atomicAdd(&stat_rep(p.s1, p.srep, p.sstride)[c], red[0][0][c] + red[0][1][c] + red[0][2][c] + red[0][3][c]);
        atomicAdd(&stat_rep(p.s2, p.srep, p.sstride)[c], red[1][0][c] + red[1][1][c] + red[1][2][c] + red[1][3][c]);
    }
}

extern "C" int mms_pool_bwd_group(const PoolBwdP* pp, int ng, hipStream_t s) { return mms_pool_bwd_group_live(pp, nullptr, ng, s); }
extern "C" int mms_pool_bwd_group_live(const PoolBwdP* pp, const unsigned* const* live, int ng, hipStream_t s) {
    const LiveTab lt = live_tab(live, ng);
    Grp<PoolBwdP> a;
    if (!grp_fill(a, pp, ng, 1)) return MMS_ERR_ARG;
    const PoolBwdP& p = *pp;
    const int Min = p.B * p.in.D * p.in.H * p.in.W;
    if (Min <= 0) return MMS_ERR_ARG;
    for (int g = 1; g < ng; ++g) {
        const PoolBwdP& q = pp[g];
        if (q.B != p.B || q.in.D != p.in.D || q.in.H != p.in.H || q.in.W != p.in.W || q.out.D != p.out.D || q.out.H != p.out.H ||
            q.out.W != p.out.W) return MMS_ERR_ARG;
    }
    if (p.in.D % 2 == 0 && p.in.H % 4 == 0 && p.in.W % 16 == 0) {
        if (p.in.W % 32 == 0) {
            MMS_LAUNCH(pool_bwd_brick_kernel<32>, dim3(p.B * (p.in.D / 2) * (p.in.H / 4) * (p.in.W / 32), 1, ng), dim3(256), 0, s, a, lt);
        } else {
            MMS_LAUNCH(pool_bwd_brick_kernel<16>, dim3(p.B * (p.in.D / 2) * (p.in.H / 4) * (p.in.W / 16), 1, ng), dim3(256), 0, s, a, lt);
        }
        return mms_check_launch();
    }
    MMS_LAUNCH(pool_bwd_kernel, dim3((Min + 63) / 64, 1, ng), dim3(256), 0, s, a, lt);
    return mms_check_launch();
}
MMS_SINGLE(mms_pool_bwd, PoolBwdP)

struct Conv0BwdWOp {
    typedef Conv0BwdWP Params;
    static constexpr int WM = 2, WN = 2, WK = 1, AMODE = LD_K1, BMODE = LD_R4;
    __device__ void step(const Params&, int) {}
    static constexpr int TM = 64, TN = 64;
    static constexpr int EXTRA = 5 * 64;
    float *A, *Bc, *Cc, *mean, *rstd;
    int k0r, mb, me;
    __device__ void setup(const Params& p, int m0_, int, int z, float* extra, int tid) {
        k0r = m0_;
        A = extra; Bc = extra + 64; Cc = extra + 128; mean = extra + 192; rstd = extra + 256;
        if (tid < 64) {
// ... 268 lines not shown
```

### multimodal_survival_prediction_amd/csrc/dn_net.hip

```cpp
#include "dn_ops.h"
#include <string.h>
#include <stdio.h>
#include <stdlib.h>

namespace {

constexpr int NB = 4;
constexpr int LAYERS[NB] = {6, 12, 24, 16};
constexpr int C0[NB] = {64, 128, 256, 512};
constexpr int CTOT[NB] = {256, 512, 1024, 1024};
constexpr int NLAYER = 58;
constexpr int NBN = 121;
constexpr int NPARAM = 364;


struct Plan {
    int B; Dims3 in, g0, g[NB];
    int M0, M[NB];
    long partial_rows;
    int R0, R[NB];
    size_t coords0, coords[NB], y0, argmax, slab[NB], dslab[NB], y1[NLAYER], wpf[NLAYER], wpb[NLAYER];
    size_t dbn_mid_l[NLAYER], dbn_in, dbn0, pooled, tab_pack, tab_bn, partial, dwp[NLAYER];
    size_t dw0_rep;
    size_t tpool[3];
    size_t stats_begin, stats_begin_packed, stats_end;
    size_t st_y0, st_slab[NB], st_y1[NLAYER];
    size_t counters;
    int cl_rt[NB], cl_rpc[NB], cl_ncl[NB];
    size_t cl_xa[NB], cl_xb[NB], cl_gst[NB], cl_tab[NB], cl_zero_begin, cl_ga, cl_gz;
    size_t b4_err;
    size_t bwd_live;
    size_t zw;
    size_t hx;
    size_t bb_y0, bb_y1[NLAYER], bb_in[NLAYER], bb_tr[3], bb_head;
    size_t total;
};

inline size_t al(size_t x) { return (x + 255) & ~(size_t)255; }

bool make_plan(Plan& P, int B, int D, int H, int W) {
    if (B <= 0 || D < 32 || H < 32 || W < 32 || (D % 32) || (H % 32) || (W % 32)) return false;
    if (D > 1023 * 2 || H > 1023 * 2 || W > 1023 * 2) return false;
    P.B = B; P.in = Dims3{D, H, W};
    P.g0 = Dims3{D / 2, H / 2, W / 2};
    P.g[0] = Dims3{D / 4, H / 4, W / 4};
    for (int b = 1; b < NB; ++b) P.g[b] = Dims3{P.g[b - 1].D / 2, P.g[b - 1].H / 2, P.g[b - 1].W / 2};
    P.M0 = B * P.g0.D * P.g0.H * P.g0.W;
    for (int b = 0; b < NB; ++b) P.M[b] = B * P.g[b].D * P.g[b].H * P.g[b].W;
    constexpr int rep_rows = 2048;
    auto reps = [](int M) { int r = 1; while (r < 8 && M / (2 * r) >= rep_rows) r *= 2; return r; };
    P.R0 = reps(P.M0);
    for (int b = 0; b < NB; ++b) P.R[b] = reps(P.M[b]);
    size_t o = 0;
    auto take = [&](size_t bytes) { size_t r = o; o = al(o + bytes); return r; };
    P.coords0 = take((size_t)P.M0 * 4);
    for (int b = 0; b < NB; ++b) P.coords[b] = take((size_t)P.M[b] * 4);
    P.y0 = take((size_t)P.M0 * 64 * 4);
    P.argmax = take((size_t)P.M[0] * 64);
    for (int b = 0; b < NB; ++b) P.slab[b] = take((size_t)P.M[b] * CTOT[b] * 4);
    for (int b = 0; b < NB; ++b) P.dslab[b] = take((size_t)P.M[b] * CTOT[b] * 4);
    int l = 0;
    for (int b = 0; b < NB; ++b)
        for (int i = 0; i < LAYERS[b]; ++i, ++l) {
            P.y1[l] = take((size_t)P.M[b] * 128 * 4);
            P.wpf[l] = take((size_t)32 * 27 * 128 * 4);
            P.wpb[l] = take((size_t)32 * 27 * 128 * 4);
        }
    {
        int l2 = 0;
        for (int b = 0; b < NB; ++b)
            for (int i = 0; i < LAYERS[b]; ++i, ++l2) P.dbn_mid_l[l2] = take((size_t)P.M[b] * 128 * 4);
    }
    size_t mx = 0;
    for (int b = 0; b < NB; ++b) { size_t v = (size_t)P.M[b] * CTOT[b] * 4; if (v > mx) mx = v; }
    P.dbn_in = take(mx);
    P.dbn0 = take((size_t)P.M0 * 64 * 4);
    P.pooled = take((size_t)B * 1024 * 4);
    {
        size_t a = (size_t)27 * (P.M[1] > 1024 ? 1024 : P.M[1]) * 128 * 4, b2 = (size_t)3 * P.M[0] * 128 * 4;
        P.partial = take(a > b2 ? a : b2);
        P.partial_rows = (long)((a > b2 ? a : b2) / (128 * 4));
    }
    P.tab_pack = take(sizeof(PackEntry) * NLAYER);
    P.tab_bn = take(sizeof(BnRunEntry) * NBN);
    P.stats_begin = o;
    for (int i = 0; i < NLAYER; ++i) P.dwp[i] = take((size_t)27 * 32 * 128 * 4);
    P.stats_begin_packed = o;
    int blk_of[NLAYER];
    { int l2 = 0; for (int b = 0; b < NB; ++b) for (int i = 0; i < LAYERS[b]; ++i) blk_of[l2++] = b; }
    P.st_y0 = take((size_t)P.R0 * 2 * 64 * 8);
    for (int b = 0; b < NB; ++b) P.st_slab[b] = take((size_t)P.R[b] * 2 * CTOT[b] * 8);
    for (int i = 0; i < NLAYER; ++i) P.st_y1[i] = take((size_t)P.R[blk_of[i]] * 2 * 128 * 8);
    P.bb_y0 = take((size_t)P.R0 * 2 * 64 * 8);
    for (int i = 0; i < NLAYER; ++i) P.bb_y1[i] = take((size_t)P.R[blk_of[i]] * 2 * 128 * 8);
    for (int i = 0; i < NLAYER; ++i) P.bb_in[i] = take((size_t)P.R[blk_of[i]] * 2 * 1024 * 8);
    for (int i = 0; i < 3; ++i) P.bb_tr[i] = take((size_t)P.R[i] * 2 * 1024 * 8);
    P.bb_head = take((size_t)2 * 1024 * 8);
    P.hx = take(256);
    P.zw = take(256);
    P.cl_zero_begin = o;
    P.cl_ga = take((size_t)2 * 8 * 256 * 8);
    P.cl_gz = take((size_t)512 * 8);
    for (int b = 0; b < NB; ++b) {
        const int vox = P.g[b].D * P.g[b].H * P.g[b].W;
        int rt = b >= 2 ? (vox <= 16 ? 1 : (vox <= 32 ? 2 : 0)) : 0;
        int spc = rt ? (16 * rt) / vox : 0;
        if (spc > B) spc = B;
        int ncl = rt ? (B + spc - 1) / spc : 0;
        if (ncl > 8 || P.R[b] != 1) rt = 0;
        P.cl_rt[b] = rt; P.cl_rpc[b] = rt ? spc * vox : 0; P.cl_ncl[b] = rt ? ncl : 0;
        P.cl_xa[b] = P.cl_xb[b] = P.cl_gst[b] = 0;
        if (rt) {
            P.cl_xa[b] = take((size_t)ncl * 8 * rt * 256 * 8);
            P.cl_xb[b] = take((size_t)ncl * 8 * rt * 512 * 8);
            P.cl_gst[b] = take((size_t)ncl * 8 * 192 * 8);
        }
    }
    P.dw0_rep = take((size_t)8 * 64 * 343 * 4);
    P.stats_end = o;
    for (int t = 0; t < 3; ++t) P.tpool[t] = take((size_t)P.M[t + 1] * CTOT[t] * 4);
    P.counters = take(4096 * 4);
    P.b4_err = take(1024);
    P.bwd_live = take(4);
    for (int b = 0; b < NB; ++b) P.cl_tab[b] = take(sizeof(B4Layer) * LAYERS[b]);
    P.total = o;
    return true;
}

struct Idx {
    int conv0 = 0, n0w = 1, n0b = 2;
    int layer[NLAYER];
    int trans[3];
    int n5w, n5b, outw, outb;
    int bn_layer1[NLAYER], bn_layer2[NLAYER], bn_trans[3], bn5, bn0 = 0;
    Idx() {
        int p = 3, q = 1, l = 0;
        for (int b = 0; b < NB; ++b) {
            for (int i = 0; i < LAYERS[b]; ++i, ++l) { layer[l] = p; p += 6; bn_layer1[l] = q++; bn_layer2[l] = q++; }
            if (b < 3) { trans[b] = p; p += 3; bn_trans[b] = q++; }
        }
        n5w = p++; n5b = p++; bn5 = q++; outw = p++; outb = p++;
    }
};
const Idx IDX;

template <class T> inline T* at(void* ws, size_t off) { return (T*)((char*)ws + off); }

inline BnSrc mk_bn(void* ws, size_t st_off, int Ctot_, const float* const* prm, int iw, const void* const* buf, int bn_ord,
                   int count, int train, int nrep) {
    BnSrc b;
    b.nrep = nrep; b.rep_stride = 2 * Ctot_;
    b.sum = at<double>(ws, st_off);
    b.sumsq = at<double>(ws, st_off) + Ctot_;
    b.rmean = buf ? (const float*)buf[3 * bn_ord] : nullptr;
    b.rvar = buf ? (const float*)buf[3 * bn_ord + 1] : nullptr;
    b.gamma = prm[iw]; b.beta = prm[iw + 1];
    b.inv_count = 1.0f / (float)count; b.eps = 1e-5f; b.train = train;
    return b;
}

}

extern "C" int mms_init_coords(int*, int, int, int, int, hipStream_t);
extern "C" int mms_pack_conv3_table_group_ex(const void* const*, int, int, uint64_t, hipStream_t);
extern "C" int mms_unpack_conv3_grads(const void*, int, hipStream_t);
extern "C" int mms_bn_running_update_group(const void* const*, int, int, float, hipStream_t);
extern "C" int mms_zero_regions_group(void* const*, int, size_t, hipStream_t);
extern "C" int mms_conv0_fwd_group_zw(const Conv0FwdP*, unsigned* const*, int, const MmsDnOpts*, hipStream_t);
extern "C" int mms_pool_fwd_group(const PoolFwdP*, int, hipStream_t);
extern "C" int mms_pool_act_group(const PoolActP*, int, hipStream_t);
extern "C" int mms_conv1_fwd_group(const Conv1FwdP*, int, const MmsDnOpts*, hipStream_t);
extern "C" int mms_conv3_fwd_group(const Conv3FwdP*, int, const MmsDnOpts*, hipStream_t);
extern "C" int mms_head_fwd_group(const HeadFwdP*, int, hipStream_t);
extern "C" int mms_conv3_bwd_data_group(const Conv3BwdDataP*, int, const MmsDnOpts*, hipStream_t);
extern "C" int mms_conv3_bwd_weight_group(const Conv3BwdWP*, int, const MmsDnOpts*, hipStream_t);
extern "C" int mms_conv1_bwd_data_group(const Conv1BwdP*, int, const MmsDnOpts*, hipStream_t);
extern "C" int mms_conv1_bwd_weight_group(const Conv1BwdP*, int, hipStream_t);
extern "C" int mms_bn_bwd_apply_group(const BnBwdApplyP*, int, hipStream_t);
extern "C" int mms_head_bwd_group(const HeadBwdP*, int, hipStream_t);
extern "C" int mms_head_bwd_sums(const HeadBwdP*, hipStream_t);
extern "C" int mms_head_bwd_apply(const HeadBwdP*, hipStream_t);
extern "C" int mms_pool_bwd_group(const PoolBwdP*, int, hipStream_t);
extern "C" int mms_conv0_bwd_weight_group(const Conv0BwdWP*, int, const MmsDnOpts*, hipStream_t);

static inline int out_features_of(const MmsDnOpts& o) { return o.out_features > 0 ? o.out_features : 128; }

#ifdef MMS_ABLATE_STEP
static inline bool dbg_skip(int bit) {
    const char* e = getenv("MMS_DEBUG_SKIP");
    if (!e) return false;
    const unsigned long long m = strtoull(e, nullptr, 0);
    static std::once_flag once;
    if (m) std::call_once(once, [m] { fprintf(stderr, "mmsurv: MMS_DEBUG_SKIP=0x%llx -- TIMING ABLATION BUILD, launches are left out of every step: RESULTS ARE WRONG\n", m); });
    return (m >> bit) & 1ull;
}
#define TRYS(bit, x) do { if (!dbg_skip(bit)) TRY(x); } while (0)
#else
#define TRYS(bit, x) TRY(x)
#endif
#define TRY(x) do { int rc_ = (x); if (rc_ != MMS_OK) { fprintf(stderr, "mmsurv: %s -> %d (dn_net.hip:%d)\n", #x, rc_, __LINE__); return rc_; } } while (0)

extern "C" int mms_dn121_workspace_bytes(int B, int D, int H, int W, size_t* bytes) {
    Plan P;
    if (!make_plan(P, B, D, H, W) || !bytes) return MMS_ERR_ARG;
    *bytes = P.total;
    return MMS_OK;
}

extern "C" int mms_dn121_region(int B, int D, int H, int W, const char* name, int index, size_t* off, size_t* bytes) {
    Plan P;
    if (!make_plan(P, B, D, H, W)) return MMS_ERR_ARG;
    auto set = [&](size_t o, size_t n) { *off = o; *bytes = n; return MMS_OK; };
    if (!strcmp(name, "y0")) return set(P.y0, (size_t)P.M0 * 64 * 4);
    if (!strcmp(name, "slab") && index >= 0 && index < NB) return set(P.slab[index], (size_t)P.M[index] * CTOT[index] * 4);
    if (!strcmp(name, "dslab") && index >= 0 && index < NB) return set(P.dslab[index], (size_t)P.M[index] * CTOT[index] * 4);
    if (!strcmp(name, "y1") && index >= 0 && index < NLAYER) {
        int b = 0, l = index;
        while (l >= LAYERS[b]) { l -= LAYERS[b]; ++b; }
        return set(P.y1[index], (size_t)P.M[b] * 128 * 4);
    }
    if (!strcmp(name, "tpool") && index >= 0 && index < 3) return set(P.tpool[index], (size_t)P.M[index + 1] * CTOT[index] * 4);
    if (!strcmp(name, "stats")) return set(P.stats_begin, P.stats_end - P.stats_begin);
    if (!strcmp(name, "b4_err")) return set(P.b4_err, 1024);
    if (!strcmp(name, "hx")) return set(P.hx, 256);
    if (!strcmp(name, "zero_words")) return set(P.zw, 256);
    if (!strcmp(name, "bwd_live")) return set(P.bwd_live, 4);
    return MMS_ERR_ARG;
}

static int dn121_init_impl(void* ws, int B, int D, int H, int W, const void* const* params,
                           const void* const* buffers, int bn_world, const MmsDnOpts* opts, hipStream_t s) {
    Plan P;
    const bool packed = opts && opts->w2_packed;
    if (!make_plan(P, B, D, H, W) || !ws || !params || !buffers || bn_world < 1) return MMS_ERR_ARG;
    if (packed) for (int l2 = 0; l2 < NLAYER; ++l2) if (!params[NPARAM + 2 * l2]) return MMS_ERR_ARG;
    TRY(mms_init_coords(at<int>(ws, P.coords0), B, P.g0.D, P.g0.H, P.g0.W, s));
    for (int b = 0; b < NB; ++b) TRY(mms_init_coords(at<int>(ws, P.coords[b]), B, P.g[b].D, P.g[b].H, P.g[b].W, s));
    (void)hipGetLastError();
    PackEntry pk[NLAYER];
    BnRunEntry bn[NBN];
    auto set_bn = [&](int ord, size_t st, int Ctot_, int C, int count, int nrep) {
        bn[ord].nrep = nrep; bn[ord].rep_stride = 2 * Ctot_;
        bn[ord].sum = at<double>(ws, st); bn[ord].sumsq = at<double>(ws, st) + Ctot_;
        bn[ord].rmean = (float*)buffers[3 * ord]; bn[ord].rvar = (float*)buffers[3 * ord + 1];
        bn[ord].nbt = (long long*)buffers[3 * ord + 2]; bn[ord].C = C; bn[ord].count = (float)count * (float)bn_world;
    };
    set_bn(0, P.st_y0, 64, 64, P.M0, P.R0);
    int l = 0;
    for (int b = 0; b < NB; ++b) {
        int C = C0[b];
        for (int i = 0; i < LAYERS[b]; ++i, ++l, C += 32) {
            pk[l].w = (const float*)params[IDX.layer[l] + 5];
            pk[l].wpf = at<float>(ws, P.wpf[l]); pk[l].wpb = at<float>(ws, P.wpb[l]);
            set_bn(IDX.bn_layer1[l], P.st_slab[b], CTOT[b], C, P.M[b], P.R[b]);
            set_bn(IDX.bn_layer2[l], P.st_y1[l], 128, 128, P.M[b], P.R[b]);
        }
        if (b < 3) set_bn(IDX.bn_trans[b], P.st_slab[b], CTOT[b], CTOT[b], P.M[b], P.R[b]);
        else set_bn(IDX.bn5, P.st_slab[b], CTOT[b], CTOT[b], P.M[b], P.R[b]);
    }
    if (hipMemsetAsync(at<void>(ws, P.counters), 0, 4096 * 4, s) != hipSuccess) return MMS_ERR_LAUNCH;
    if (hipMemsetAsync(at<void>(ws, P.b4_err), 0, 1024, s) != hipSuccess) return MMS_ERR_LAUNCH;
    B4Layer clt[NLAYER];
    for (int li = 0; li < NLAYER; ++li) {
        const int ip = IDX.layer[li], o1 = IDX.bn_layer1[li], o2 = IDX.bn_layer2[li];
        clt[li] = B4Layer{(const float*)params[ip], (const float*)params[ip + 1], (const float*)params[ip + 2],
                          (const float*)params[ip + 3], (const float*)params[ip + 4],
                          packed ? (const float*)params[ip + 5] : at<float>(ws, P.wpf[li]),
                          packed ? (const float*)params[NPARAM + 2 * li] : at<float>(ws, P.wpb[li]),
                          (const float*)buffers[3 * o1], (const float*)buffers[3 * o1 + 1], (const float*)buffers[3 * o2], (const float*)buffers[3 * o2 + 1],
                          at<float>(ws, P.y1[li]), at<double>(ws, P.st_y1[li]), at<float>(ws, P.dbn_mid_l[li]), at<double>(ws, P.bb_y1[li])};
    }
    hipError_t e0 = hipSuccess;
    {
        int l0 = 0;
        for (int b = 0; b < NB; ++b) {
            const hipError_t e = hipMemcpyAsync(at<void>(ws, P.cl_tab[b]), clt + l0, sizeof(B4Layer) * LAYERS[b], hipMemcpyHostToDevice, s);
            if (e != hipSuccess) e0 = e;
            l0 += LAYERS[b];
        }
    }
    if (e0 != hipSuccess) return MMS_ERR_LAUNCH;
    hipError_t e1 = hipMemcpyAsync(at<void>(ws, P.tab_pack), pk, sizeof(pk), hipMemcpyHostToDevice, s);
    hipError_t e2 = hipMemcpyAsync(at<void>(ws, P.tab_bn), bn, sizeof(bn), hipMemcpyHostToDevice, s);
    hipError_t e3 = hipStreamSynchronize(s);
    if (e1 != hipSuccess || e2 != hipSuccess || e3 != hipSuccess) {
        fprintf(stderr, "mms_dn121_init: memcpy/sync failed: %s / %s / %s\n", hipGetErrorString(e1), hipGetErrorString(e2), hipGetErrorString(e3));
        return MMS_ERR_LAUNCH;
    }
    return MMS_OK;
}

extern "C" int mms_dn121_init(void* ws, int B, int D, int H, int W, const void* const* params,
                              const void* const* buffers, const MmsDnOpts* opts, hipStream_t s) {
    return dn121_init_impl(ws, B, D, H, W, params, buffers, 1, opts, s);
}
extern "C" int mms_dn121_init_sync(void* ws, int B, int D, int H, int W, const void* const* params,
                                   const void* const* buffers, int bn_world, const MmsDnOpts* opts, hipStream_t s) {
    return dn121_init_impl(ws, B, D, H, W, params, buffers, bn_world, opts, s);
}

static int split_target(const MmsDnOpts& o) {
    return o.split_wgs > 0 ? o.split_wgs : 256;
}
static int conv3_nsplit(int M, int ng, long cap_rows, const Dims3& g, const MmsDnOpts& o) {
    if (mms_conv3_small_jn(M, ng, g, o)) return 1;
    const long tiles = (long)((M + 31) / 32) * ng;
    if (tiles >= 256 && tiles >= split_target(o)) return 1;
    long ns = (split_target(o) + tiles - 1) / tiles;
    if (ns > 27) ns = 27;
    if (ns < 1) ns = 1;
    int tpw = (int)((27 + ns - 1) / ns);
    while (tpw < 27 && (long)((27 + tpw - 1) / tpw) * M > cap_rows) ++tpw;
    return (27 + tpw - 1) / tpw;
}

static bool cluster_block(const Plan& P, int b, const MmsDnOpts& o, int pass) {
    if (b < 2 || !P.cl_rt[b]) return false;
    if (b == 2) return pass == 0 && o.persist_b3 > 0;
    if (pass == 1 && P.M[3] > 16) return false;
    return pass == 0 ? o.persist_b4 >= 0 : o.persist_b4 == 0;
}
static bool conv3_frag_block(const Plan& P, int b, int ng, const MmsDnOpts& o) {
    return b < NB - 1 && mms_conv3_small_jn(P.M[b], ng, P.g[b], o) != 0 && (o.w2_packed || !cluster_block(P, b, o, 0));
}
static bool fuse_block(const Plan& P, int b, int ng, const MmsDnOpts& o) {
    if (o.fuse_layers < 0 || b != 2 || ng > MMS_FUSE_MAXG || P.M[b] > 128 || P.R[b] != 1 || cluster_block(P, b, o, 0)) return false;
    if (mms_conv3_small_jn(P.M[b], ng, P.g[b], o) != 1 || !conv3_frag_block(P, b, ng, o) || (o.c3s_ring > 0 && o.c3s_ring != 6)) return false;
    Conv1FwdP q{};
    q.M = P.M[b]; q.N = 128; q.K = CTOT[b] - 32; q.ldx = CTOT[b];
    return mms_conv1_small_ok(q, ng, o);
}
static uint64_t conv3_fragmask(const Plan& P, int ng, const MmsDnOpts& o) {
    uint64_t m = 0;
    int l = 0;
    for (int b = 0; b < NB; ++b)
        for (int i = 0; i < LAYERS[b]; ++i, ++l) if (conv3_frag_block(P, b, ng, o)) m |= 1ull << l;
    return m;
}

extern "C" int mms_dn121_w2_fragmask(int B, int D, int H, int W, const MmsDnOpts* opts, uint64_t* mask) {
    Plan P;
    if (!make_plan(P, B, D, H, W) || !mask) return MMS_ERR_ARG;
    *mask = conv3_fragmask(P, 1, mms_opts(opts));
    return MMS_OK;
}

struct Ctx {
    void* ws; const float* x; const float* const* prm; const void* const* buf; float* out;
    const float* dout; float* const* grd;
};
struct Dp {
    int bn_world = 1; mms_sync_fn hook = nullptr; void* user = nullptr;
    int b_hi = NB - 1, b_lo = 0;
    bool staged = false;
};
#define SYNC(ptr, nrep, rstride, ncols, pstride) do { if (dp.hook) { int rc_ = dp.hook(dp.user, (ptr), (nrep), (long)(rstride), (ncols), (long)(pstride), s); \
    if (rc_ != MMS_OK) { fprintf(stderr, "mmsurv: statistics all-reduce hook failed (dn_net.hip:%d)\n", __LINE__); return MMS_ERR_LAUNCH; } } } while (0)
#define FOR_G for (int g = 0; g < ng; ++g)

static int dn121_forward_impl(const Ctx* cx, int ng, int B, int D, int H, int W, int ldo, int train, const MmsDnOpts* opts, hipStream_t s, const Dp& dp = Dp()) {
    const MmsDnOpts o = mms_opts(opts);
    const int nout = out_features_of(o);
    Plan P;
    if (!make_plan(P, B, D, H, W) || ng < 1 || ng > MMS_MAX_GROUP || nout > 4096 || ldo < nout) return MMS_ERR_ARG;
    if ((dp.hook || dp.bn_world > 1) && (ng != 1 || !train)) return MMS_ERR_ARG;
    const int bw = dp.bn_world;
    FOR_G if (!cx[g].ws || !cx[g].x || !cx[g].prm || !cx[g].out) return MMS_ERR_ARG;
    const void* tabs[MMS_MAX_GROUP];
    const bool packed = o.w2_packed != 0;
    if (train) {
        void* regs[MMS_MAX_GROUP];
        const size_t zb = packed ? P.stats_begin_packed : P.stats_begin;
        FOR_G regs[g] = at<void>(cx[g].ws, zb);
        TRY(mms_zero_regions_group(regs, ng, P.stats_end - zb, s));
    }
    if (!packed) {
        FOR_G tabs[g] = at<void>(cx[g].ws, P.tab_pack);
        TRY(mms_pack_conv3_table_group_ex(tabs, ng, NLAYER, conv3_fragmask(P, ng, o), s));
    }
    auto st = [&](void* ws, size_t off, int Ctot_, int coff, bool sq) -> double* {
        return train ? at<double>(ws, off) + (sq ? Ctot_ : 0) + coff : nullptr;
    };
    const bool cl_ok = !dp.hook && dp.bn_world == 1;
    const bool dupz = o.dup_zero >= 0 && cl_ok && B >= 2 && B <= 32;
    const int zbps = (P.g0.D / 4) * (P.g0.H / 4) * (P.g0.W / 4);
    if (!train && (dupz || (cl_ok && fuse_block(P, 2, ng, o)))) {
        void* regs[MMS_MAX_GROUP];
        FOR_G regs[g] = at<void>(cx[g].ws, P.hx);
        TRY(mms_zero_regions_group(regs, ng, 512, s));
    }
    {
        Conv0FwdP c0[MMS_MAX_GROUP];
        PoolFwdP pf[MMS_MAX_GROUP];
        FOR_G {
            const Ctx& c = cx[g];
            c0[g] = Conv0FwdP{c.x, P.in, P.g0, at<int>(c.ws, P.coords0), P.M0, c.prm[IDX.conv0], at<float>(c.ws, P.y0),
                              st(c.ws, P.st_y0, 64, 0, false), st(c.ws, P.st_y0, 64, 0, true)};
            c0[g].srep = P.R0; c0[g].sstride = 2 * 64;
            pf[g] = PoolFwdP{at<float>(c.ws, P.y0), P.g0, P.g[0], B, at<float>(c.ws, P.slab[0]), CTOT[0], at<uint8_t>(c.ws, P.argmax),
                             mk_bn(c.ws, P.st_y0, 64, c.prm, IDX.n0w, c.buf, IDX.bn0, P.M0 * bw, train, P.R0),
                             st(c.ws, P.st_slab[0], CTOT[0], 0, false), st(c.ws, P.st_slab[0], CTOT[0], 0, true)};
            pf[g].srep = P.R[0]; pf[g].sstride = 2 * CTOT[0];
        }
        unsigned* zws[MMS_MAX_GROUP];
        FOR_G zws[g] = at<unsigned>(cx[g].ws, P.zw);
        TRYS(28, mms_conv0_fwd_group_zw(c0, dupz ? zws : nullptr, ng, &o, s));
        SYNC(at<double>(cx[0].ws, P.st_y0), P.R0, 2 * 64, 64, 64);
        TRYS(28, mms_pool_fwd_group(pf, ng, s));
        SYNC(at<double>(cx[0].ws, P.st_slab[0]), P.R[0], 2 * CTOT[0], 64, CTOT[0]);
    }
    if (!train && cl_ok && (cluster_block(P, 2, o, 0) || cluster_block(P, 3, o, 0))) {
        void* regs[MMS_MAX_GROUP];
        FOR_G regs[g] = at<void>(cx[g].ws, P.cl_zero_begin);
        TRY(mms_zero_regions_group(regs, ng, P.stats_end - P.cl_zero_begin, s));
    }
    int l = 0;
    for (int b = 0; b < NB; ++b) {
        int C = C0[b];
        if (cl_ok && cluster_block(P, b, o, 0)) {
            ClFwdP q[MMS_MAX_GROUP];
            FOR_G {
                const Ctx& c = cx[g];
                q[g] = ClFwdP{at<B4Layer>(c.ws, P.cl_tab[b]), LAYERS[b], C0[b], at<float>(c.ws, P.slab[b]), CTOT[b], at<double>(c.ws, P.st_slab[b]),
                              at<int>(c.ws, P.coords[b]), P.g[b], P.M[b], P.cl_rpc[b], P.cl_ncl[b], train, 1e-5f,
                              at<unsigned long long>(c.ws, P.cl_xa[b]), at<unsigned long long>(c.ws, P.cl_xb[b]), at<unsigned long long>(c.ws, P.cl_gst[b]),
                              at<unsigned>(c.ws, P.b4_err)};
            }
            TRYS(32, mms_cl_fwd_group(q, ng, s));
            l += LAYERS[b];
            C += 32 * LAYERS[b];
        } else {
            const int ns3 = conv3_nsplit(P.M[b], ng, P.partial_rows, P.g[b], o);
            const bool frag3 = conv3_frag_block(P, b, ng, o);
            auto mk_c1 = [&](const Ctx& c, int l_, int C_) {
                const int ip = IDX.layer[l_];
                Conv1FwdP q{at<float>(c.ws, P.slab[b]), CTOT[b], P.M[b], C_, c.prm[ip + 2], 128, at<float>(c.ws, P.y1[l_]), 128,
                            mk_bn(c.ws, P.st_slab[b], CTOT[b], c.prm, ip, c.buf, IDX.bn_layer1[l_], P.M[b] * bw, train, P.R[b]),
                            st(c.ws, P.st_y1[l_], 128, 0, false), st(c.ws, P.st_y1[l_], 128, 0, true), 0, Dims3{0, 0, 0}};
                q.srep = P.R[b]; q.sstride = 2 * 128;
                if (o.conv1_ksplit >= 0 && (long)((P.M[b] + 31) / 32) * 4 * ng <= 128 && C_ >= 256 && (long)((C_ + 127) / 128) * P.M[b] <= P.partial_rows) {
                    q.partial = at<float>(c.ws, P.partial); q.ksplit = (C_ + 127) / 128; q.counters = at<unsigned>(c.ws, P.counters);
                }
                return q;
            };
            const bool fuse = cl_ok && fuse_block(P, b, ng, o);
            for (int i = 0; i < LAYERS[b]; ++i, ++l, C += 32) {
                const int ip = IDX.layer[l];
                Conv1FwdP c1[MMS_MAX_GROUP];
                Conv3FwdP c3[MMS_MAX_GROUP];
                FOR_G {
                    const Ctx& c = cx[g];
                    c1[g] = mk_c1(c, l, C);
                    const float* wp3 = !packed ? at<float>(c.ws, P.wpf[l]) : (frag3 ? c.prm[NPARAM + 2 * l + 1] : c.prm[ip + 5]);
                    c3[g] = Conv3FwdP{at<float>(c.ws, P.y1[l]), at<int>(c.ws, P.coords[b]), P.g[b], P.M[b], wp3,
                                      at<float>(c.ws, P.slab[b]) + C, CTOT[b],
                                      mk_bn(c.ws, P.st_y1[l], 128, c.prm, ip + 3, c.buf, IDX.bn_layer2[l], P.M[b] * bw, train, P.R[b]),
                                      st(c.ws, P.st_slab[b], CTOT[b], C, false), st(c.ws, P.st_slab[b], CTOT[b], C, true),
                                      ns3 > 1 ? at<float>(c.ws, P.partial) : nullptr, ns3};
                    c3[g].srep = P.R[b]; c3[g].sstride = 2 * CTOT[b]; c3[g].wfrag = frag3 ? 1 : 0;
                    c3[g].zwords = dupz ? at<unsigned>(c.ws, P.zw) : nullptr; c3[g].zbps = zbps;
                }
                if (!fuse || i == 0) {
                    TRYS(b, mms_conv1_fwd_group(c1, ng, &o, s));
                    SYNC(at<double>(cx[0].ws, P.st_y1[l]), P.R[b], 2 * 128, 128, 128);
                }
                if (fuse && i + 1 < LAYERS[b]) {
                    Conv1FwdP n1[MMS_MAX_GROUP];
                    unsigned* fl[MMS_MAX_GROUP];
                    unsigned* er[MMS_MAX_GROUP];
                    FOR_G { n1[g] = mk_c1(cx[g], l + 1, C + 32); fl[g] = at<unsigned>(cx[g].ws, P.hx) + l; er[g] = at<unsigned>(cx[g].ws, P.b4_err); }
                    TRYS(4 + b, mms_c3s_c1s_fwd(c3, n1, fl, er, ng, s));
                } else {
                    TRYS(4 + b, mms_conv3_fwd_group(c3, ng, &o, s));
                    SYNC(at<double>(cx[0].ws, P.st_slab[b]) + C, P.R[b], 2 * CTOT[b], 32, CTOT[b]);
                }
            }
        }
        if (b < 3) {
            const int ip = IDX.trans[b];
            Conv1FwdP t[MMS_MAX_GROUP];
            PoolActP pa[MMS_MAX_GROUP];
            const bool pre = o.trans_prepass >= 0;
            FOR_G {
                const Ctx& c = cx[g];
                const BnSrc bnt = mk_bn(c.ws, P.st_slab[b], CTOT[b], c.prm, ip, c.buf, IDX.bn_trans[b], P.M[b] * bw, train, P.R[b]);
                pa[g] = PoolActP{at<float>(c.ws, P.slab[b]), CTOT[b], CTOT[b], bnt, P.g[b], P.M[b + 1], at<float>(c.ws, P.tpool[b]), CTOT[b]};
                t[g] = Conv1FwdP{pre ? at<float>(c.ws, P.tpool[b]) : at<float>(c.ws, P.slab[b]), CTOT[b], P.M[b + 1], CTOT[b], c.prm[ip + 2], CTOT[b] / 2,
                                 at<float>(c.ws, P.slab[b + 1]), CTOT[b + 1], pre ? BnSrc{} : bnt,
                                 st(c.ws, P.st_slab[b + 1], CTOT[b + 1], 0, false), st(c.ws, P.st_slab[b + 1], CTOT[b + 1], 0, true), pre ? 0 : 1, pre ? Dims3{0, 0, 0} : P.g[b]};
                t[g].srep = P.R[b + 1]; t[g].sstride = 2 * CTOT[b + 1];
            }
            if (pre) TRYS(30, mms_pool_act_group(pa, ng, s));
            TRYS(30, mms_conv1_fwd_group(t, ng, &o, s));
            SYNC(at<double>(cx[0].ws, P.st_slab[b + 1]), P.R[b + 1], 2 * CTOT[b + 1], CTOT[b] / 2, CTOT[b + 1]);
        }
    }
    HeadFwdP hd[MMS_MAX_GROUP];
    FOR_G {
        const Ctx& c = cx[g];
        hd[g] = HeadFwdP{at<float>(c.ws, P.slab[3]), CTOT[3], 1024, B, P.M[3] / B,
                         mk_bn(c.ws, P.st_slab[3], CTOT[3], c.prm, IDX.n5w, c.buf, IDX.bn5, P.M[3] * bw, train, P.R[3]),
                         c.prm[IDX.outw], c.prm[IDX.outb], nout, at<float>(c.ws, P.pooled), c.out, ldo};
    }
    TRY(mms_head_fwd_group(hd, ng, s));
    if (train) {
        bool all = true;
        FOR_G { all = all && cx[g].buf; tabs[g] = at<void>(cx[g].ws, P.tab_bn); }
        if (all) TRY(mms_bn_running_update_group(tabs, ng, NBN, 0.1f, s));
    }
    return MMS_OK;
}

static int dn121_backward_impl(const Ctx* cx, int ng, int B, int D, int H, int W, int lddout, const MmsDnOpts* opts, hipStream_t s, hipStream_t side,
                               hipEvent_t ev_fork, hipEvent_t ev_join, const Dp& dp = Dp()) {
    const MmsDnOpts o = mms_opts(opts);
    const int nout = out_features_of(o);
    if (nout > 4096 || lddout < nout) return MMS_ERR_ARG;
    hipStream_t sw = side ? side : s;
    bool side_pending = false;
    Plan P;
    if (!make_plan(P, B, D, H, W) || ng < 1 || ng > MMS_MAX_GROUP) return MMS_ERR_ARG;
    FOR_G if (!cx[g].ws || !cx[g].x || !cx[g].prm || !cx[g].dout || !cx[g].grd) return MMS_ERR_ARG;
    if ((dp.hook || dp.bn_world > 1) && ng != 1) return MMS_ERR_ARG;
    if (dp.b_hi < dp.b_lo || dp.b_hi >= NB || dp.b_lo < 0) return MMS_ERR_ARG;
    const int bnw = dp.bn_world;
    const bool sync = dp.hook != nullptr || bnw > 1;
    const bool packed = o.w2_packed != 0;
    auto bbsrc = [&](void* ws, size_t off, int stride, int nrep) { return BnBwd{at<double>(ws, off), at<double>(ws, off) + stride, nrep, 2 * stride}; };
    const bool skip_dead = o.skip_dead_bwd >= 0 && !sync && !dp.staged && dp.b_hi == NB - 1;
    auto lv = [&](const Ctx& c) -> unsigned* { return skip_dead ? at<unsigned>(c.ws, P.bwd_live) : nullptr; };
    const unsigned* lvs[MMS_MAX_GROUP];
    FOR_G lvs[g] = lv(cx[g]);
    if (dp.b_hi == NB - 1) {
        HeadBwdP hb[MMS_MAX_GROUP];
        unsigned* hlive[MMS_MAX_GROUP];
        FOR_G {
            const Ctx& c = cx[g];
            hb[g] = HeadBwdP{c.dout, lddout, at<float>(c.ws, P.pooled), at<float>(c.ws, P.slab[3]), CTOT[3], 1024, B, P.M[3] / B,
                             mk_bn(c.ws, P.st_slab[3], CTOT[3], c.prm, IDX.n5w, nullptr, 0, P.M[3] * bnw, 1, P.R[3]), c.prm[IDX.outw], nout,
                             c.grd[IDX.outw], c.grd[IDX.outb], c.grd[IDX.n5w], c.grd[IDX.n5b], at<float>(c.ws, P.dslab[3]), CTOT[3]};
            hlive[g] = lv(c);
        }
        if (sync) {
            hb[0].ext_sums = at<double>(cx[0].ws, P.bb_head);
            TRY(mms_head_bwd_sums(hb, s));
            SYNC(at<double>(cx[0].ws, P.bb_head), 1, 2 * 1024, 1024, 1024);
            TRY(mms_head_bwd_apply(hb, s));
        } else {
            TRY(mms_head_bwd_group_live(hb, hlive, ng, s));
        }
    }
    const bool batch_w = o.batch_w >= 0 && !side;
    Conv3BwdWP bwq[MMS_MAX_GROUP];
    Conv1BwdP c1q[MMS_MAX_GROUP];
    int nq = 0;
    int nq_limit = MMS_MAX_GROUP;
    const bool wtab = batch_w && o.wgrad_tab >= 0 && !sync && !dp.staged && ng <= MMS_WGRAD_MAX_MODELS;
    MmsWgradModel wmod[MMS_WGRAD_MAX_MODELS];
    MmsWgradMember wmem[MMS_WGRAD_MAX_MEMBERS];
    MmsWgradShape wsh{};
    int nwq = 0;
    auto flush_w = [&](int b) -> int {
        if (nwq > 0) {
            TRYS(12 + b, mms_wgrad_tab_group_live(wmod, lvs, ng, wmem, nwq, &wsh, 1, s));
            TRYS(16 + b, mms_wgrad_tab_group_live(wmod, lvs, ng, wmem, nwq, &wsh, 2, s));
            nwq = 0;
        }
        if (nq == 0) return MMS_OK;
        TRYS(12 + b, mms_conv3_bwd_weight_group(bwq, nq, &o, s));
        TRYS(16 + b, mms_conv1_bwd_weight_group(c1q, nq, s));
        nq = 0;
        return MMS_OK;
    };
    int l = NLAYER;
    for (int b = NB - 1; b > dp.b_hi; --b) l -= LAYERS[b];
    for (int b = dp.b_hi; b >= dp.b_lo; --b) {
        int C = CTOT[b];
        const int M = P.M[b];
        const bool defer = batch_w && (b > 0 || o.batch_w == 0) && 2 * ng <= MMS_MAX_GROUP;
        int ngw_blk = ng;
        if (defer) {
            if (b > 0) ngw_blk = MMS_MAX_GROUP / ng * ng;
            else { const int nl = (LAYERS[b] * ng + MMS_MAX_GROUP - 1) / MMS_MAX_GROUP; ngw_blk = (LAYERS[b] + nl - 1) / nl * ng; }
        }
        nq_limit = ngw_blk;
        const int fuse_rows = o.fuse_apply_rows > 0 ? o.fuse_apply_rows : (o.conv1_small_bwd < 0 ? 32 : 128);
        const bool fuse_apply = M <= fuse_rows && M <= 128 && !sync;
        const bool b4_bwd = b == 3 && !sync && dp.bn_world == 1 && defer && fuse_apply && cluster_block(P, 3, o, 1);
        if (b4_bwd) {
            ClBwdP q[MMS_MAX_GROUP];
            FOR_G {
                const Ctx& c = cx[g];
                q[g] = ClBwdP{at<B4Layer>(c.ws, P.cl_tab[3]), LAYERS[3], C0[3], at<float>(c.ws, P.slab[3]), at<float>(c.ws, P.dslab[3]), CTOT[3],
                              at<double>(c.ws, P.st_slab[3]), at<int>(c.ws, P.coords[3]), P.g[3], M, 1e-5f,
                              at<unsigned long long>(c.ws, P.cl_ga), at<unsigned long long>(c.ws, P.cl_gz), at<unsigned>(c.ws, P.b4_err), {}, {}};
                for (int i = 0; i < LAYERS[3]; ++i) {
                    const int ip = IDX.layer[NLAYER - LAYERS[3] + i];
                    q[g].dg1[i] = (float*)c.grd[ip]; q[g].db1[i] = (float*)c.grd[ip + 1];
                }
                q[g].live = lv(c);
            }
            TRYS(33, mms_cl_bwd_group(q, ng, s));
        }
        for (int i = LAYERS[b] - 1; i >= 0; --i) {
            --l; C -= 32;
            const int ip = IDX.layer[l];
            Conv3BwdDataP bd[MMS_MAX_GROUP];
            Conv3BwdWP bw[MMS_MAX_GROUP];
            Conv1BwdP c1[MMS_MAX_GROUP];
            BnBwdApplyP ap[MMS_MAX_GROUP];
            const int ns3 = conv3_nsplit(M, ng, P.partial_rows, P.g[b], o);
            const int ngw = ngw_blk;
            const int ms3 = mms_conv3w_msplit(M, ngw, o);
            int ms1 = M > 1024 ? M / 256 : M / 128; if (ms1 < 1) ms1 = 1; if (ms1 > 32) ms1 = 32;
            { const int dv = o.ms1_div > 0 ? o.ms1_div : (ngw >= 4 ? 2 : 1); if (dv > 1) { ms1 = ms1 / dv; if (ms1 < 1) ms1 = 1; } }
            FOR_G {
                const Ctx& c = cx[g];
                float* slab = at<float>(c.ws, P.slab[b]);
                float* dslab = at<float>(c.ws, P.dslab[b]);
                float* dmid = at<float>(c.ws, P.dbn_mid_l[l]);
                const BnSrc bn1 = mk_bn(c.ws, P.st_slab[b], CTOT[b], c.prm, ip, nullptr, 0, M * bnw, 1, P.R[b]);
                const BnSrc bn2 = mk_bn(c.ws, P.st_y1[l], 128, c.prm, ip + 3, nullptr, 0, M * bnw, 1, P.R[b]);
                bd[g] = Conv3BwdDataP{dslab + C, CTOT[b], at<int>(c.ws, P.coords[b]), P.g[b], M, packed ? c.prm[NPARAM + 2 * l] : at<float>(c.ws, P.wpb[l]),
                                      at<float>(c.ws, P.y1[l]), bn2, dmid,
                                      at<double>(c.ws, P.bb_y1[l]), at<double>(c.ws, P.bb_y1[l]) + 128,
                                      ns3 > 1 ? at<float>(c.ws, P.partial) : nullptr, ns3};
                bd[g].srep = P.R[b]; bd[g].sstride = 2 * 128; bd[g].wfrag = conv3_frag_block(P, b, ng, o) ? 1 : 0; bd[g].live = lv(c);
                bw[g] = Conv3BwdWP{at<float>(c.ws, P.y1[l]), at<int>(c.ws, P.coords[b]), P.g[b], M, bn2, dslab + C, CTOT[b],
                                   packed ? c.grd[ip + 5] : at<float>(c.ws, P.dwp[l]), ms3, packed ? 2 : 1, lv(c)};
                Conv1BwdP& q = c1[g];
                q = Conv1BwdP{};
                q.dyraw = dmid; q.lddy = 128;
                q.y = at<float>(c.ws, P.y1[l]); q.ldy = 128;
                q.bn_out = bn2; q.bb_out = bbsrc(c.ws, P.bb_y1[l], 128, P.R[b]); q.has_bn_out = 1;
                q.M = M; q.N = 128;
                q.x = slab; q.ldx = CTOT[b]; q.K = C; q.bn_in = bn1;
                q.w = c.prm[ip + 2]; q.pool = 0; q.in = Dims3{0, 0, 0};
                q.dw = c.grd[ip + 2];
                q.dbn = at<float>(c.ws, P.dbn_in); q.lddbn = CTOT[b];
                q.s1 = at<double>(c.ws, P.bb_in[l]); q.s2 = at<double>(c.ws, P.bb_in[l]) + 1024;
                q.srep = P.R[b]; q.sstride = 2 * 1024;
                q.msplit = ms1; q.dgamma_out = c.grd[ip + 3]; q.dbeta_out = c.grd[ip + 4];
                q.live = lv(c);
                if (fuse_apply) { q.fuse_dx = dslab; q.fuse_lddx = CTOT[b]; q.fuse_accumulate = 1; q.fuse_dgamma = c.grd[ip]; q.fuse_dbeta = c.grd[ip + 1]; }
                ap[g] = BnBwdApplyP{at<float>(c.ws, P.dbn_in), CTOT[b], slab, CTOT[b], dslab, CTOT[b], M, C, bn1,
                                    bbsrc(c.ws, P.bb_in[l], 1024, P.R[b]), 1, c.grd[ip], c.grd[ip + 1], lv(c)};
            }
            if (side && side_pending) {
                if (hipStreamWaitEvent(s, ev_join, 0) != hipSuccess) return MMS_ERR_LAUNCH;
                side_pending = false;
            }
            if (!b4_bwd) {
                TRYS(8 + b, mms_conv3_bwd_data_group(bd, ng, &o, s));
                SYNC(at<double>(cx[0].ws, P.bb_y1[l]), P.R[b], 2 * 128, 128, 128);
            }
            if (defer && wtab && b > 0) {
                if (nwq + ng > MMS_WGRAD_MAX_MEMBERS) TRY(flush_w(b));
                if (nwq == 0) {
                    FOR_G wmod[g] = MmsWgradModel{at<B4Layer>(cx[g].ws, P.cl_tab[b]), at<float>(cx[g].ws, P.slab[b]), at<float>(cx[g].ws, P.dslab[b]),
                                                  at<int>(cx[g].ws, P.coords[b]), at<double>(cx[g].ws, P.st_slab[b]), M, P.g[b], P.R[b]};
                    wsh = MmsWgradShape{CTOT[b], C0[b], ms3, ms1, packed ? 2 : 1, M * bnw};
                }
                FOR_G {
                    if (!mms_bn_aligned16(bw[g].bn)) return MMS_ERR_ARG;
                    wmem[nwq++] = MmsWgradMember{bw[g].dw, c1[g].dw, c1[g].dgamma_out, c1[g].dbeta_out, g, i};
                }
            } else if (defer) {
                if (nq + ng > nq_limit) TRY(flush_w(b));
                FOR_G { bwq[nq] = bw[g]; c1q[nq] = c1[g]; ++nq; }
            } else {
                if (side) {
                    if (hipEventRecord(ev_fork, s) != hipSuccess || hipStreamWaitEvent(side, ev_fork, 0) != hipSuccess) return MMS_ERR_LAUNCH;
                }
                TRYS(12 + b, mms_conv3_bwd_weight_group(bw, ng, &o, sw));
                TRYS(16 + b, mms_conv1_bwd_weight_group(c1, ng, sw));
                if (side) {
                    if (hipEventRecord(ev_join, side) != hipSuccess) return MMS_ERR_LAUNCH;
                    side_pending = true;
                }
            }
            if (b4_bwd) continue;
            TRYS(20 + b, mms_conv1_bwd_data_group(c1, ng, &o, s));
            SYNC(at<double>(cx[0].ws, P.bb_in[l]), P.R[b], 2 * 1024, C, 1024);
            if (!fuse_apply) TRYS(24 + b, mms_bn_bwd_apply_group(ap, ng, s));
        }
        TRY(flush_w(b));
        if (side && side_pending) {
            if (hipStreamWaitEvent(s, ev_join, 0) != hipSuccess) return MMS_ERR_LAUNCH;
            side_pending = false;
        }
        if (b > 0) {
            const int t = b - 1, ip = IDX.trans[t], Kp = CTOT[t], Mp = P.M[t];
            int ms1 = M / 256; if (ms1 < 1) ms1 = 1; if (ms1 > 32) ms1 = 32;
            Conv1BwdP c1[MMS_MAX_GROUP];
            BnBwdApplyP ap[MMS_MAX_GROUP];
            FOR_G {
                const Ctx& c = cx[g];
                const BnSrc bnt = mk_bn(c.ws, P.st_slab[t], CTOT[t], c.prm, ip, nullptr, 0, Mp * bnw, 1, P.R[t]);
                Conv1BwdP& q = c1[g];
                q = Conv1BwdP{};
                q.dyraw = at<float>(c.ws, P.dslab[b]); q.lddy = CTOT[b]; q.y = nullptr; q.ldy = 0; q.has_bn_out = 0;
                q.bn_out = bnt; q.bb_out = BnBwd{nullptr, nullptr, 0, 0};
                q.M = M; q.N = Kp / 2;
                q.x = at<float>(c.ws, P.slab[t]); q.ldx = CTOT[t]; q.K = Kp; q.bn_in = bnt;
                q.w = c.prm[ip + 2]; q.pool = 1; q.in = P.g[t];
                q.dw = c.grd[ip + 2];
                q.dbn = at<float>(c.ws, P.dbn_in); q.lddbn = CTOT[t];
                q.s1 = at<double>(c.ws, P.bb_tr[t]); q.s2 = at<double>(c.ws, P.bb_tr[t]) + 1024;
                q.srep = P.R[t]; q.sstride = 2 * 1024;
                q.msplit = ms1; q.dgamma_out = nullptr; q.dbeta_out = nullptr; q.live = lv(c);
                ap[g] = BnBwdApplyP{at<float>(c.ws, P.dbn_in), CTOT[t], at<float>(c.ws, P.slab[t]), CTOT[t], at<float>(c.ws, P.dslab[t]), CTOT[t],
                                    Mp, Kp, bnt, bbsrc(c.ws, P.bb_tr[t], 1024, P.R[t]), 0, c.grd[ip], c.grd[ip + 1], lv(c)};
            }
            if (o.trans_prepass >= 0) {
                Conv1BwdP cw[MMS_MAX_GROUP];
                FOR_G { cw[g] = c1[g]; cw[g].x = at<float>(cx[g].ws, P.tpool[t]); cw[g].pool = 0; cw[g].in = Dims3{0, 0, 0}; cw[g].bn_in = BnSrc{}; }
                TRYS(31, mms_conv1_bwd_weight_group(cw, ng, s));
            } else TRYS(31, mms_conv1_bwd_weight_group(c1, ng, s));
            TRYS(31, mms_conv1_bwd_data_group(c1, ng, &o, s));
            SYNC(at<double>(cx[0].ws, P.bb_tr[t]), P.R[t], 2 * 1024, Kp, 1024);
            TRYS(31, mms_bn_bwd_apply_group(ap, ng, s));
        } else {
            int ms0 = P.M0 / 1024; if (ms0 < 1) ms0 = 1; if (ms0 > 64) ms0 = 64;
            PoolBwdP pb[MMS_MAX_GROUP];
            Conv0BwdWP cw[MMS_MAX_GROUP];
            FOR_G {
                const Ctx& c = cx[g];
                const BnSrc bn0 = mk_bn(c.ws, P.st_y0, 64, c.prm, IDX.n0w, nullptr, 0, P.M0 * bnw, 1, P.R0);
                pb[g] = PoolBwdP{at<float>(c.ws, P.dslab[0]), CTOT[0], at<uint8_t>(c.ws, P.argmax), P.g[0], P.g0, B, at<float>(c.ws, P.y0), bn0,
                                 at<float>(c.ws, P.dbn0), at<double>(c.ws, P.bb_y0), at<double>(c.ws, P.bb_y0) + 64, at<int>(c.ws, P.coords0)};
                pb[g].srep = P.R0; pb[g].sstride = 2 * 64;
                cw[g] = Conv0BwdWP{at<float>(c.ws, P.dbn0), at<float>(c.ws, P.y0), bn0, bbsrc(c.ws, P.bb_y0, 64, P.R0), c.x, P.in, P.g0,
                                   at<int>(c.ws, P.coords0), P.M0, c.grd[IDX.conv0], ms0, c.grd[IDX.n0w], c.grd[IDX.n0b],
                                   at<float>(c.ws, P.dw0_rep), 8, lv(c)};
            }
            TRYS(29, mms_pool_bwd_group_live(pb, lvs, ng, s));
            SYNC(at<double>(cx[0].ws, P.bb_y0), P.R0, 2 * 64, 64, 64);
            TRYS(29, mms_conv0_bwd_weight_group(cw, ng, &o, s));
        }
    }
    if (side && side_pending) {
        if (hipStreamWaitEvent(s, ev_join, 0) != hipSuccess) return MMS_ERR_LAUNCH;
    }
    {
        static_assert(NLAYER == 58, "UnpackGroup is sized for DenseNet121");
        int l0 = 0, nl = 0;
        for (int b = 0; b < NB; ++b) { if (b < dp.b_lo) l0 += LAYERS[b]; else if (b <= dp.b_hi) nl += LAYERS[b]; }
        if (nl == 0 || packed) return MMS_OK;
        const float* scr[MMS_MAX_GROUP];
        float* dwt[MMS_MAX_GROUP][NLAYER];
        float* const* dwp_[MMS_MAX_GROUP];
        if (P.dwp[1] - P.dwp[0] != (size_t)27 * 32 * 128 * 4) return MMS_ERR_ARG;
        FOR_G {
            scr[g] = at<float>(cx[g].ws, P.dwp[l0]);
            for (int i = 0; i < nl; ++i) dwt[g][i] = cx[g].grd[IDX.layer[l0 + i] + 5];
            dwp_[g] = dwt[g];
        }
        TRY(mms_unpack_conv3_grads_group_live(scr, dwp_, lvs, ng, nl, s));
    }
    return MMS_OK;
}

extern "C" int mms_dn121_forward(void* ws, int B, int D, int H, int W, const float* x, const void* const* params_,
                                 const void* const* buffers, float* out, int ldo, int train, const MmsDnOpts* opts, hipStream_t s) {
    Ctx c{ws, x, (const float* const*)params_, buffers, out, nullptr, nullptr};
    return dn121_forward_impl(&c, 1, B, D, H, W, ldo, train, opts, s);
}
extern "C" int mms_dn121_backward(void* ws, int B, int D, int H, int W, const float* x, const void* const* params,
                                  const float* dout, int lddout, void* const* grads, const MmsDnOpts* opts, hipStream_t s) {
    Ctx c{ws, x, (const float* const*)params, nullptr, nullptr, dout, (float* const*)grads};
    return dn121_backward_impl(&c, 1, B, D, H, W, lddout, opts, s, nullptr, nullptr, nullptr);
}
extern "C" int mms_dn121_backward_mt(void* ws, int B, int D, int H, int W, const float* x, const void* const* params,
                                     const float* dout, int lddout, void* const* grads, const MmsDnOpts* opts, hipStream_t s, hipStream_t side,
                                     hipEvent_t ev_fork, hipEvent_t ev_join) {
    if (!side || !ev_fork || !ev_join) return MMS_ERR_ARG;
    Ctx c{ws, x, (const float* const*)params, nullptr, nullptr, dout, (float* const*)grads};
    return dn121_backward_impl(&c, 1, B, D, H, W, lddout, opts, s, side, ev_fork, ev_join);
}

extern "C" int mms_conv0_bwd_data_group(const Conv0BwdDataP*, int, hipStream_t);
static int dn121_input_grad_impl(const Ctx* cx, int ng, int B, int D, int H, int W, int lddout, const MmsDnOpts* opts, hipStream_t s) {
// ... 145 lines not shown
```

Measured before the change: 3622.

## Skip duplicate all-zero samples in conv3 backward data and weight kernels

```diff
diff --git a/include/mmsurv.h b/include/mmsurv.h
--- a/include/mmsurv.h
+++ b/include/mmsurv.h
@@ -47,6 +47,7 @@
     int skip_dead_bwd;
     int c0_zero_skip;
     int dup_zero;
+    int dup_zero_bwd;
 } MmsDnOpts;
 
 typedef struct BnSrc {
@@ -150,6 +151,7 @@
     int srep; int sstride;
     int wfrag;
     const unsigned* live;
+    const unsigned* dup;
 } Conv3BwdDataP;
 
 typedef struct Conv3BwdWP {
@@ -160,6 +162,7 @@
     int msplit;
     int dw_layout;
     const unsigned* live;
+    const unsigned* dup;
 } Conv3BwdWP;
 
 #define MMS_WGRAD_MAX_MODELS 5
@@ -556,6 +559,8 @@
                         const MmsWgradShape* shape, int which, hipStream_t s);
 int mms_bn_bwd_apply_group(const BnBwdApplyP* p, int ng, hipStream_t s);
 int mms_head_bwd_group(const HeadBwdP* p, int ng, hipStream_t s);
+int mms_head_bwd_group_dup(const HeadBwdP* p, unsigned* const* live_out, const unsigned* const* zwords, int zbps, unsigned* const* dup_out,
+                           int ng, hipStream_t s);
 int mms_pool_bwd_group(const PoolBwdP* p, int ng, hipStream_t s);
 int mms_conv0_bwd_weight_group(const Conv0BwdWP* p, int ng, const MmsDnOpts* opts, hipStream_t s);
 int mms_pack_conv3_table_group(const void* const* tables_dev, int ng, int nlayers, hipStream_t s);
diff --git a/multimodal_survival_prediction_amd/csrc/common.h b/multimodal_survival_prediction_amd/csrc/common.h
--- a/multimodal_survival_prediction_amd/csrc/common.h
+++ b/multimodal_survival_prediction_amd/csrc/common.h
@@ -20,7 +20,11 @@
 }
 #define MMS_SINGLE(name, T) extern "C" int name(const T* p, hipStream_t s) { return name##_group(p, 1, s); }
 #define MMS_SINGLE_O(name, T) extern "C" int name(const T* p, hipStream_t s) { return name##_group(p, 1, nullptr, s); }
+#ifdef MMS_DUP_ZERO_BWD_DEFAULT
+static inline MmsDnOpts mms_opts(const MmsDnOpts* o) { MmsDnOpts r = o ? *o : MmsDnOpts{}; if (r.dup_zero_bwd == 0) r.dup_zero_bwd = MMS_DUP_ZERO_BWD_DEFAULT; return r; }
+#else
 static inline MmsDnOpts mms_opts(const MmsDnOpts* o) { return o ? *o : MmsDnOpts{}; }
+#endif
 
 
 __device__ __forceinline__ void xcd_place(int& gi, int& bx) {
@@ -53,9 +57,8 @@
     const int lane = threadIdx.x & 63;
     return (zw && lane < B) ? __hip_atomic_load(zw + lane, __ATOMIC_RELAXED, __HIP_MEMORY_SCOPE_AGENT) : 0xffffffffu;
 }
-__device__ __forceinline__ bool dup_resolve(unsigned word, unsigned zbps, int B, int tps, int mode, int X, int q, int sl, int& tile, DupPlan& pl) {
+__device__ __forceinline__ bool dup_plan(unsigned zmask, int B, int tps, int mode, int X, int q, int sl, int& tile, DupPlan& pl) {
     pl.dups = 0; pl.rep = 0;
-    const unsigned zmask = (unsigned)__builtin_amdgcn_readfirstlane((int)(unsigned)__ballot(word == zbps));
     if (__popc(zmask) < 2) return true;
     const int rep = __ffs((int)zmask) - 1;
     const unsigned dmask = zmask & ~(1u << rep);
@@ -77,6 +80,25 @@
     }
     if (s == rep) { pl.dups = dmask; pl.rep = rep; }
     return true;
+}
+__device__ __forceinline__ bool dup_resolve(unsigned word, unsigned zbps, int B, int tps, int mode, int X, int q, int sl, int& tile, DupPlan& pl) {
+    const unsigned zmask = (unsigned)__builtin_amdgcn_readfirstlane((int)(unsigned)__ballot(word == zbps));
+    return dup_plan(zmask, B, tps, mode, X, q, sl, tile, pl);
+}
+
+__device__ __forceinline__ unsigned dupm_issue(const unsigned* w) {
+    return w ? __hip_atomic_load(w, __ATOMIC_RELAXED, __HIP_MEMORY_SCOPE_AGENT) : 0u;
+}
+__device__ __forceinline__ unsigned dupm_mask(unsigned word, int B) {
+    const unsigned m = (unsigned)__builtin_amdgcn_readfirstlane((int)word) & (B >= 32 ? 0xffffffffu : (1u << B) - 1u);
+    return __popc(m) < 2 ? 0u : m;
+}
+__device__ __forceinline__ bool dup_resolve_mask(unsigned mask, int B, int tps, int X, int q, int sl, int& tile, DupPlan& pl) {
+    return dup_plan(mask, B, tps, 0, X, q, sl, tile, pl);
+}
+__device__ __forceinline__ int nth_bit(unsigned keep, int n) {
+    for (; n > 0; --n) keep &= keep - 1u;
+    return __ffs((int)keep) - 1;
 }
 
 __device__ __forceinline__ unsigned live_issue(const unsigned* w) {
diff --git a/multimodal_survival_prediction_amd/csrc/dn_bwd.hip b/multimodal_survival_prediction_amd/csrc/dn_bwd.hip
--- a/multimodal_survival_prediction_amd/csrc/dn_bwd.hip
+++ b/multimodal_survival_prediction_amd/csrc/dn_bwd.hip
@@ -186,12 +186,14 @@
 #define C3D_BP 36
 #define C3D_MAXHALO 17
 #define C3D_PIN() do { if constexpr (PIN) { asm volatile("" ::: "memory"); __builtin_amdgcn_sched_barrier(0); } } while (0)
+struct DupBwdArgs { int on, B, tps, rps; };
 template <bool PIN>
-__global__ __launch_bounds__(256) __attribute__((amdgpu_waves_per_eu(3, 3))) void conv3_bwd_data_mt_kernel(const Grp<Conv3BwdDataP> grp) {
-    int gi, bx;
-    xcd_place(gi, bx);
+__global__ __launch_bounds__(256) __attribute__((amdgpu_waves_per_eu(3, 3))) void conv3_bwd_data_mt_kernel(const Grp<Conv3BwdDataP> grp, const DupBwdArgs da) {
+    int gi, bx, xX, xq, xsl;
+    xcd_place_parts(gi, bx, xX, xq, xsl);
     const Conv3BwdDataP& p = grp.p[gi];
     const unsigned alive = live_issue(p.live);
+    const unsigned dword = da.on ? dupm_issue(p.dup) : 0u;
     const float* __restrict__ dz = p.dz;
     const float* __restrict__ wpb = p.wpb;
     const float* __restrict__ y1 = p.y1;
@@ -199,24 +201,29 @@
     const int M = p.M, lddz = p.lddz, W = p.g.W, HW = p.g.H * p.g.W;
     extern __shared__ __attribute__((aligned(16))) float smem[];
     const int tid = threadIdx.x, lane = tid & 63, wave = tid >> 6, li = lane & 31, kq = lane >> 5;
-    const int m0 = bx * 32, halo = W + 1, nrows = 32 + 2 * halo;
+    const int halo = W + 1, nrows = 32 + 2 * halo;
+    int m0 = bx * 32;
     const int cin = 32 * wave + li;
     float mu, rstd, ga, be;
     bn_consts1(p.bn, cin, mu, rstd, ga, be);
-    const int myrow = m0 + li;
-    const int mycoord = p.coords[myrow < M ? myrow : 0];
+    int myrow, mycoord;
     constexpr int NR = (32 + 2 * C3D_MAXHALO + 31) / 32;
     float4 wv[3][NR];
     const int wr = tid >> 3, wc = (tid & 7) * 4;
-#pragma unroll
-    for (int kd = 0; kd < 3; ++kd)
-#pragma unroll
-        for (int i = 0; i < NR; ++i) {
-            const int r = wr + 32 * i, src = m0 - (kd - 1) * HW - halo + r;
-            const bool ok = r < nrows && src >= 0 && src < M;
-            const float4 v = *(const float4*)(dz + (size_t)(ok ? src : 0) * lddz + wc);
-            wv[kd][i] = ok ? v : make_float4(0.f, 0.f, 0.f, 0.f);
-        }
+    auto wload = [&]() __attribute__((always_inline)) {
+        myrow = m0 + li;
+        mycoord = p.coords[myrow < M ? myrow : 0];
+#pragma unroll
+        for (int kd = 0; kd < 3; ++kd)
+#pragma unroll
+            for (int i = 0; i < NR; ++i) {
+                const int r = wr + 32 * i, src = m0 - (kd - 1) * HW - halo + r;
+                const bool ok = r < nrows && src >= 0 && src < M;
+                const float4 v = *(const float4*)(dz + (size_t)(ok ? src : 0) * lddz + wc);
+                wv[kd][i] = ok ? v : make_float4(0.f, 0.f, 0.f, 0.f);
+            }
+    };
+    wload();
     const float* wl = wpb + (size_t)cin * 864 + 4 * kq;
     float4 b[3][4];
     auto bload = [&](float4 (&bb)[4], int tap) __attribute__((always_inline)) {
@@ -226,6 +233,14 @@
     bload(b[0], 0);
     bload(b[1], 1);
     if (live_dead(alive)) return;
+    DupPlan dup{0u, 0};
+    if (da.on) {
+        if (const unsigned dmask = dupm_mask(dword, da.B)) {
+            int tile = bx;
+            if (!dup_resolve_mask(dmask, da.B, da.tps, xX, xq, xsl, tile, dup)) return;
+            if (tile != bx) { m0 = tile * 32; wload(); }
+        }
+    }
 #pragma unroll
     for (int kd = 0; kd < 3; ++kd)
 #pragma unroll
@@ -287,11 +302,14 @@
             const float pre = fmaf(ga, xh, be);
             const float g = pre > 0.f ? acc[r] + acc2[r] : 0.f;
             dbn[(size_t)m * 128 + cin] = g;
+            for (unsigned dm = dup.dups; dm; dm &= dm - 1u)
+                dbn[((size_t)m + (size_t)((__ffs((int)dm) - 1 - dup.rep) * da.rps)) * 128 + cin] = g;
             s1 += g; s2 += (double)g * xh;
         }
     }
     s1 += __shfl_xor(s1, 32);
     s2 += __shfl_xor(s2, 32);
+    if (dup.dups) { const double mul = (double)(1 + __popc(dup.dups)); s1 *= mul; s2 *= mul; }
     if (kq == 0) {
         atomicAdd(&stat_rep(p.s1, p.srep, p.sstride)[cin], s1);
         atomicAdd(&stat_rep(p.s2, p.srep, p.sstride)[cin], s2);
@@ -303,13 +321,24 @@
     const int min32 = o.conv3_mt32_min > 0 ? o.conv3_mt32_min : 256;
     return M >= 1024 && (long)((M + 31) / 32) * ng >= min32;
 }
+template <class P>
+static DupBwdArgs conv3_dup_bwd_args(const P* pp, int ng, const MmsDnOpts& o, int which) {
+    const P& p = *pp;
+    const long rps = (long)p.g.D * p.g.H * p.g.W;
+    DupBwdArgs da{0, 0, 0, 0};
+    if (o.dup_zero_bwd < 0 || (o.dup_zero_bwd != 0 && o.dup_zero_bwd != which)) return da;
+    if (rps <= 0 || rps % 32 != 0 || p.M % rps != 0 || p.M / rps > 32 || p.M / rps < 2) return da;
+    for (int g = 0; g < ng; ++g) if (!pp[g].dup) return da;
+    da.on = 1; da.B = (int)(p.M / rps); da.tps = (int)(rps / 32); da.rps = (int)rps;
+    return da;
+}
 template <bool PIN>
-static int launch_conv3_bwd_data_mt(const Conv3BwdDataP* pp, int ng, hipStream_t s) {
+static int launch_conv3_bwd_data_mt(const Conv3BwdDataP* pp, int ng, const MmsDnOpts& o, hipStream_t s) {
     const Conv3BwdDataP& p = *pp;
     const int smem = (3 * (32 + 2 * (p.g.W + 1)) + 1) * C3D_BP * (int)sizeof(float);
     Grp<Conv3BwdDataP> a;
     grp_fill(a, pp, ng, 1);
-    MMS_LAUNCH((conv3_bwd_data_mt_kernel<PIN>), dim3((p.M + 31) / 32, 1, ng), dim3(256), smem, s, a);
+    MMS_LAUNCH((conv3_bwd_data_mt_kernel<PIN>), dim3((p.M + 31) / 32, 1, ng), dim3(256), smem, s, a, conv3_dup_bwd_args(pp, ng, o, 1));
     return mms_check_launch();
 }
 
@@ -337,7 +366,7 @@
     }
     if (conv3_bwd_data_mt_ok(p.M, ng, p.g, o)) {
         for (int g = 0; g < ng; ++g) if (pp[g].lddz % 4 != 0 || ((uintptr_t)pp[g].dz & 15) != 0) return MMS_ERR_ARG;
-        return (long)((p.M + 31) / 32) * ng <= 768 ? launch_conv3_bwd_data_mt<true>(pp, ng, s) : launch_conv3_bwd_data_mt<false>(pp, ng, s);
+        return (long)((p.M + 31) / 32) * ng <= 768 ? launch_conv3_bwd_data_mt<true>(pp, ng, o, s) : launch_conv3_bwd_data_mt<false>(pp, ng, o, s);
     }
     if (mms_conv3_small_jn(p.M, ng, p.g, o)) return mms_c3s_bwd_data(pp, ng, o, s);
     return launch_tile_gemm<Conv3BwdDataOp<false>>(pp, ng, dim3((p.M + 31) / 32, 1, 1), s);
@@ -483,7 +512,7 @@
 #define C3W_AP 132
 #define C3W_BP 36
 #define C3W_STAGE (34 * C3W_AP + 32 * C3W_BP)
-__global__ __launch_bounds__(256) __attribute__((amdgpu_waves_per_eu(2, 3))) void conv3_bwdw_mt_kernel(const Grp<Conv3BwdWP> grp) {
+__global__ __launch_bounds__(256) __attribute__((amdgpu_waves_per_eu(2, 3))) void conv3_bwdw_mt_kernel(const Grp<Conv3BwdWP> grp, const DupBwdArgs da) {
     int gi, z;
     {
         const int flat = blockIdx.z, nflat = gridDim.z, zdim = grp.zdim, pairs = nflat / 9, ms = zdim / 9;
@@ -495,6 +524,7 @@
     }
     const Conv3BwdWP& p = grp.p[gi];
     const unsigned alive = live_issue(p.live);
+    const unsigned dword = da.on ? dupm_issue(p.dup) : 0u;
     extern __shared__ __attribute__((aligned(16))) float smem[];
     float2* vf = (float2*)(smem + 2 * C3W_STAGE);
     const int tid = threadIdx.x, lane = tid & 63, wave = tid >> 6, li = lane & 31, h = lane >> 5;
@@ -502,22 +532,40 @@
     const int offdh = ((kd - 1) * p.g.H + (kh - 1)) * p.g.W;
     int mc = (p.M + p.msplit - 1) / p.msplit;
     mc = (mc + 31) & ~31;
-    const int mb = chunk * mc, me = mb + mc < p.M ? mb + mc : p.M;
-    if (mb >= me) return;
+    int mb = chunk * mc, me = mb + mc < p.M ? mb + mc : p.M;
+    if (!da.on && mb >= me) return;
     const int c0 = (tid & 31) * 4;
     float mean[4], sc[4], beta[4];
     bn_consts4(p.bn, c0, mean, sc, beta);
     if (live_dead(alive)) return;
+    unsigned keep = 0u;
+    int rep = -1;
+    float mult = 1.f;
+    if (da.on) {
+        if (const unsigned dmask = dupm_mask(dword, da.B)) {
+            rep = __ffs((int)dmask) - 1;
+            const unsigned dups = dmask & ~(1u << rep);
+            keep = (da.B >= 32 ? 0xffffffffu : (1u << da.B) - 1u) & ~dups;
+            mult = (float)__popc(dmask);
+            const int Mc = p.M - __popc(dups) * da.rps;
+            mc = (((Mc + p.msplit - 1) / p.msplit) + 31) & ~31;
+            mb = chunk * mc; me = mb + mc < Mc ? mb + mc : Mc;
+        }
+        if (mb >= me) return;
+    }
+    auto rowof = [&](int c) __attribute__((always_inline)) { return keep ? nth_bit(keep, c / da.rps) * da.rps + c % da.rps : c; };
     for (int j = tid; j < mc; j += 256) {
-        const unsigned mk = (mb + j < me) ? tap_mask9(p.coords[mb + j], p.g, false) : 0u;
+        const unsigned mk = (mb + j < me) ? tap_mask9(p.coords[rowof(mb + j)], p.g, false) : 0u;
         vf[j] = make_float2(mk & 64u ? 1.f : 0.f, mk & 256u ? 1.f : 0.f);
     }
     const unsigned selb = (1u << kd) | (8u << kh);
 
     float4 ra[5], rb;
     unsigned oka = 0;
-    bool okb = false;
-    auto gload = [&](int r0) __attribute__((always_inline)) {
+    float zb = 0.f;
+    auto gload = [&](int cr0) __attribute__((always_inline)) {
+        const int r0 = rowof(cr0), rend = r0 + (me - cr0);
+        const float scl = keep && r0 / da.rps == rep ? mult : 1.f;
         oka = 0;
 #pragma unroll
         for (int i = 0; i < 5; ++i) {
@@ -527,8 +575,8 @@
             ra[i] = ok ? *(const float4*)(p.y1 + (size_t)src * 128 + c0) : make_float4(0.f, 0.f, 0.f, 0.f);
         }
         const int m = r0 + (tid >> 3);
-        rb = m < me ? *(const float4*)(p.dz + (size_t)m * p.lddz + (tid & 7) * 4) : make_float4(0.f, 0.f, 0.f, 0.f);
-        okb = m < me && (tap_mask9(p.coords[m], p.g, false) & selb) == selb;
+        rb = m < rend ? *(const float4*)(p.dz + (size_t)m * p.lddz + (tid & 7) * 4) : make_float4(0.f, 0.f, 0.f, 0.f);
+        zb = m < rend && (tap_mask9(p.coords[m], p.g, false) & selb) == selb ? scl : 0.f;
     };
     auto sstore = [&](float* st) __attribute__((always_inline)) {
 #pragma unroll
@@ -541,7 +589,6 @@
                                 zf * fmaxf(bn_apply(ra[i].z, mean[2], sc[2], beta[2]), 0.f), zf * fmaxf(bn_apply(ra[i].w, mean[3], sc[3], beta[3]), 0.f));
             }
         }
-        const float zb = okb ? 1.f : 0.f;
         *(float4*)&st[34 * C3W_AP + (tid >> 3) * C3W_BP + (tid & 7) * 4] = make_float4(zb * rb.x, zb * rb.y, zb * rb.z, zb * rb.w);
     };
     f32x16 acc0, acc1, acc2;
@@ -637,7 +684,7 @@
         constexpr int smem = (2 * C3W_STAGE + 2 * 1024) * (int)sizeof(float);
         Grp<Conv3BwdWP> a;
         if (!grp_fill(a, pp, ng, 9 * p.msplit)) return MMS_ERR_ARG;
-        MMS_LAUNCH(conv3_bwdw_mt_kernel, dim3(1, 1, 9 * p.msplit * ng), dim3(256), smem, s, a);
+        MMS_LAUNCH(conv3_bwdw_mt_kernel, dim3(1, 1, 9 * p.msplit * ng), dim3(256), smem, s, a, conv3_dup_bwd_args(pp, ng, o, 2));
         return mms_check_launch();
     }
     return launch_tile_gemm<Conv3BwdWOp>(pp, ng, dim3(1, 1, 27 * p.msplit), s);
@@ -1147,15 +1194,33 @@
     }
 }
 #define HEAD_LIVE_SCAN 16384
-__global__ __launch_bounds__(256) void head_bwd_w_kernel(const Grp<HeadBwdP> grp, const LiveTab lt) {
+struct DupOutTab { const unsigned* zw[MMS_MAX_GROUP]; unsigned* out[MMS_MAX_GROUP]; unsigned zbps; };
+__global__ __launch_bounds__(256) void head_bwd_w_kernel(const Grp<HeadBwdP> grp, const LiveTab lt, const DupOutTab dt) {
     const HeadBwdP& p = grp.p[blockIdx.z];
     unsigned* const live_out = (unsigned*)lt.w[blockIdx.z];
-    if (blockIdx.x == 0 && live_out) {
+    unsigned* const dup_out = dt.out[blockIdx.z];
+    if (blockIdx.x == 0 && (live_out || dup_out)) {
+        __shared__ unsigned nzrows[4];
         const int n_el = p.B * p.N;
-        int any = n_el > HEAD_LIVE_SCAN;
-        if (!any) for (int i = threadIdx.x; i < n_el; i += 256) any |= p.dout[(i / p.N) * p.lddout + i % p.N] != 0.0f;
-        any = __syncthreads_or(any);
-        if (threadIdx.x == 0) __hip_atomic_store(live_out, any ? 1u : 0u, __ATOMIC_RELAXED, __HIP_MEMORY_SCOPE_AGENT);
+        const bool scan = n_el <= HEAD_LIVE_SCAN;
+        const unsigned* zw = dt.zw[blockIdx.z];
+        const bool dup_ok = dup_out && zw && scan && p.B <= 32 && dt.zbps > 0;
+        const unsigned word = (dup_ok && (int)threadIdx.x < p.B) ? zw[threadIdx.x] : 0xffffffffu;
+        unsigned nz = 0;
+        if (scan) for (int i = threadIdx.x; i < n_el; i += 256) nz |= (p.dout[(i / p.N) * p.lddout + i % p.N] != 0.0f ? 1u : 0u) << ((i / p.N) & 31);
+        if (dup_ok) {
+            unsigned w = nz;
+#pragma unroll
+            for (int o = 32; o > 0; o >>= 1) w |= (unsigned)__shfl_xor((int)w, o, 64);
+            if ((threadIdx.x & 63) == 0) nzrows[threadIdx.x >> 6] = w;
+        }
+        const int any = __syncthreads_or(!scan || nz != 0u);
+        if (threadIdx.x == 0 && live_out) __hip_atomic_store(live_out, any ? 1u : 0u, __ATOMIC_RELAXED, __HIP_MEMORY_SCOPE_AGENT);
+        if (threadIdx.x < 64 && dup_out) {
+            unsigned d = dup_ok ? (unsigned)__ballot(word == dt.zbps) & ~(nzrows[0] | nzrows[1] | nzrows[2] | nzrows[3]) : 0u;
+            if (__popc(d) < 2) d = 0u;
+            if (threadIdx.x == 0) __hip_atomic_store(dup_out, d, __ATOMIC_RELAXED, __HIP_MEMORY_SCOPE_AGENT);
+        }
     }
     const int idx = blockIdx.x * 256 + threadIdx.x;
     if (idx >= p.N * p.C) return;
@@ -1169,8 +1234,13 @@
         p.dbias[n] += d;
     }
 }
-extern "C" int mms_head_bwd_group(const HeadBwdP* pp, int ng, hipStream_t s) { return mms_head_bwd_group_live(pp, nullptr, ng, s); }
+static_assert(sizeof(Grp<HeadBwdP>) + sizeof(LiveTab) + sizeof(DupOutTab) <= 4096, "kernel-argument segment");
+extern "C" int mms_head_bwd_group(const HeadBwdP* pp, int ng, hipStream_t s) { return mms_head_bwd_group_dup(pp, nullptr, nullptr, 0, nullptr, ng, s); }
 extern "C" int mms_head_bwd_group_live(const HeadBwdP* pp, unsigned* const* live_out, int ng, hipStream_t s) {
+    return mms_head_bwd_group_dup(pp, live_out, nullptr, 0, nullptr, ng, s);
+}
+extern "C" int mms_head_bwd_group_dup(const HeadBwdP* pp, unsigned* const* live_out, const unsigned* const* zwords, int zbps, unsigned* const* dup_out,
+                                      int ng, hipStream_t s) {
     Grp<HeadBwdP> a;
     if (!grp_fill(a, pp, ng, 1)) return MMS_ERR_ARG;
     const HeadBwdP& p = *pp;
@@ -1179,8 +1249,11 @@
         const HeadBwdP& q = pp[g];
         if (q.B != p.B || q.C != p.C || q.N != p.N || q.V != p.V) return MMS_ERR_ARG;
     }
+    DupOutTab dt{};
+    dt.zbps = zbps > 0 ? (unsigned)zbps : 0u;
+    for (int g = 0; dup_out && g < ng; ++g) { dt.out[g] = dup_out[g]; dt.zw[g] = zwords ? zwords[g] : nullptr; }
     MMS_LAUNCH(head_bwd_feat_kernel, dim3((p.C + 63) / 64, 1, ng), dim3(256), 0, s, a);
-    MMS_LAUNCH(head_bwd_w_kernel, dim3((p.N * p.C + 255) / 256, 1, ng), dim3(256), 0, s, a, live_tab((const unsigned* const*)live_out, ng));
+    MMS_LAUNCH(head_bwd_w_kernel, dim3((p.N * p.C + 255) / 256, 1, ng), dim3(256), 0, s, a, live_tab((const unsigned* const*)live_out, ng), dt);
     return mms_check_launch();
 }
 MMS_SINGLE(mms_head_bwd, HeadBwdP)
@@ -1232,7 +1305,7 @@
     Grp<HeadBwdP> a;
     if (!grp_fill(a, pp, 1, 1)) return MMS_ERR_ARG;
     MMS_LAUNCH(head_bwd_apply_kernel, dim3((pp->C + 255) / 256), dim3(256), 0, s, *pp);
-    MMS_LAUNCH(head_bwd_w_kernel, dim3((pp->N * pp->C + 255) / 256, 1, 1), dim3(256), 0, s, a, LiveTab{});
+    MMS_LAUNCH(head_bwd_w_kernel, dim3((pp->N * pp->C + 255) / 256, 1, 1), dim3(256), 0, s, a, LiveTab{}, DupOutTab{});
     return mms_check_launch();
 }
 
diff --git a/multimodal_survival_prediction_amd/csrc/dn_net.hip b/multimodal_survival_prediction_amd/csrc/dn_net.hip
--- a/multimodal_survival_prediction_amd/csrc/dn_net.hip
+++ b/multimodal_survival_prediction_amd/csrc/dn_net.hip
@@ -30,6 +30,7 @@
     size_t cl_xa[NB], cl_xb[NB], cl_gst[NB], cl_tab[NB], cl_zero_begin, cl_ga, cl_gz;
     size_t b4_err;
     size_t bwd_live;
+    size_t bwd_dup;
     size_t zw;
     size_t hx;
     size_t bb_y0, bb_y1[NLAYER], bb_in[NLAYER], bb_tr[3], bb_head;
@@ -122,6 +123,7 @@
     P.counters = take(4096 * 4);
     P.b4_err = take(1024);
     P.bwd_live = take(4);
+    P.bwd_dup = take(4);
     for (int b = 0; b < NB; ++b) P.cl_tab[b] = take(sizeof(B4Layer) * LAYERS[b]);
     P.total = o;
     return true;
@@ -225,6 +227,7 @@
     if (!strcmp(name, "hx")) return set(P.hx, 256);
     if (!strcmp(name, "zero_words")) return set(P.zw, 256);
     if (!strcmp(name, "bwd_live")) return set(P.bwd_live, 4);
+    if (!strcmp(name, "bwd_dup")) return set(P.bwd_dup, 4);
     return MMS_ERR_ARG;
 }
 
@@ -531,15 +534,19 @@
     auto lv = [&](const Ctx& c) -> unsigned* { return skip_dead ? at<unsigned>(c.ws, P.bwd_live) : nullptr; };
     const unsigned* lvs[MMS_MAX_GROUP];
     FOR_G lvs[g] = lv(cx[g]);
+    const bool dup_bwd = skip_dead && o.dup_zero_bwd >= 0 && o.dup_zero >= 0 && dp.bn_world == 1 && B >= 2 && B <= 32;
+    auto dv = [&](const Ctx& c) -> unsigned* { return dup_bwd ? at<unsigned>(c.ws, P.bwd_dup) : nullptr; };
     if (dp.b_hi == NB - 1) {
         HeadBwdP hb[MMS_MAX_GROUP];
         unsigned* hlive[MMS_MAX_GROUP];
+        unsigned* hdup[MMS_MAX_GROUP];
+        const unsigned* hzw[MMS_MAX_GROUP];
         FOR_G {
             const Ctx& c = cx[g];
             hb[g] = HeadBwdP{c.dout, lddout, at<float>(c.ws, P.pooled), at<float>(c.ws, P.slab[3]), CTOT[3], 1024, B, P.M[3] / B,
                              mk_bn(c.ws, P.st_slab[3], CTOT[3], c.prm, IDX.n5w, nullptr, 0, P.M[3] * bnw, 1, P.R[3]), c.prm[IDX.outw], nout,
                              c.grd[IDX.outw], c.grd[IDX.outb], c.grd[IDX.n5w], c.grd[IDX.n5b], at<float>(c.ws, P.dslab[3]), CTOT[3]};
-            hlive[g] = lv(c);
+            hlive[g] = lv(c); hdup[g] = dv(c); hzw[g] = at<unsigned>(c.ws, P.zw);
         }
         if (sync) {
             hb[0].ext_sums = at<double>(cx[0].ws, P.bb_head);
@@ -547,7 +554,7 @@
             SYNC(at<double>(cx[0].ws, P.bb_head), 1, 2 * 1024, 1024, 1024);
             TRY(mms_head_bwd_apply(hb, s));
         } else {
-            TRY(mms_head_bwd_group_live(hb, hlive, ng, s));
+            TRY(mms_head_bwd_group_dup(hb, hlive, hzw, (P.g0.D / 4) * (P.g0.H / 4) * (P.g0.W / 4), dup_bwd ? hdup : nullptr, ng, s));
         }
     }
     const bool batch_w = o.batch_w >= 0 && !side;
@@ -626,8 +633,9 @@
                                       at<double>(c.ws, P.bb_y1[l]), at<double>(c.ws, P.bb_y1[l]) + 128,
                                       ns3 > 1 ? at<float>(c.ws, P.partial) : nullptr, ns3};
                 bd[g].srep = P.R[b]; bd[g].sstride = 2 * 128; bd[g].wfrag = conv3_frag_block(P, b, ng, o) ? 1 : 0; bd[g].live = lv(c);
+                bd[g].dup = b == 0 ? dv(c) : nullptr;
                 bw[g] = Conv3BwdWP{at<float>(c.ws, P.y1[l]), at<int>(c.ws, P.coords[b]), P.g[b], M, bn2, dslab + C, CTOT[b],
-                                   packed ? c.grd[ip + 5] : at<float>(c.ws, P.dwp[l]), ms3, packed ? 2 : 1, lv(c)};
+                                   packed ? c.grd[ip + 5] : at<float>(c.ws, P.dwp[l]), ms3, packed ? 2 : 1, lv(c), b == 0 ? dv(c) : nullptr};
                 Conv1BwdP& q = c1[g];
                 q = Conv1BwdP{};
                 q.dyraw = dmid; q.lddy = 128;
```

New measurement: 3789 (median of 6 runs). 1.05x the previous value.
